# dbolya/yolact

Measured on AMD Instinct MI355X. Metric: images/sec (550x550, batch 8 per GPU), YOLACT yolact_resnet50 forward + Detect (Fast NMS), higher is better.
Workload: dtype f32 (fp32 in / fp32 accumulate / fp32 out; 92 % of the GEMM time on fp16x2 tiles = every fp32 operand as two fp16 pieces by round to nearest (22 significant bits + 2 signs: exact for ~2/3 of all fp32 values, one fp32 ulp otherwise), 3 exact piece products per product on the fp16 matrix pipe; measure

## Files before the change

### include/yolact_amd.h

```cpp
#ifndef YOLACT_AMD_H
#define YOLACT_AMD_H
#include <stddef.h>
#include <stdint.h>

#ifdef __cplusplus
extern "C" {
#endif

#define YMI_ABI_VERSION 9

#define YMI_EFORMAT (-4)
#define YMI_EUNSUPPORTED (-5)

enum { YMI_ACT_NONE = 0, YMI_ACT_RELU = 1, YMI_ACT_LEAKY01 = 2, YMI_ACT_TANH = 3, YMI_ACT_SIGMOID = 4 };
enum { YMI_RES_NONE = 0, YMI_RES_ADD = 1, YMI_RES_BILINEAR = 2 };

typedef struct {
  int32_t n0, n1;
  int32_t act;
  int32_t row_stride;
  int64_t batch_stride;
  float *ptr;
} ymi_conv_seg;

typedef struct {
  const float *x;
  const float *w;
  const float *scale;
  const float *bias;
  const float *res;
  int32_t B, H, W, Cin, ldx;
  int32_t Ho, Wo, Cout;
  int32_t kh, kw, stride, pad;
  int32_t Kpad;
  int32_t res_mode;
  int32_t res_ld;
  int32_t res_H, res_W;
  int32_t res_after_act;
  int32_t nseg;
  int32_t tile;
  int32_t cin_alg;
  int32_t split_k;
  ymi_conv_seg seg[3];
  const void *w_x3;
  float *split_ws;
  int32_t cout_alg;
  int32_t _pad2;
  const void *w_h2;
  const float *scale_h2;
  const float *winv_h2;
  const float *x_amax;
  float *y_amax;
  float x_amax_mul;
  int32_t _pad3;
} ymi_conv_desc;

enum { YMI_TILE_AUTO = 0, YMI_TILE_128x128 = 1, YMI_TILE_128x64 = 2, YMI_TILE_64x64 = 3, YMI_TILE_128x32 = 4,
       YMI_TILE_64x128 = 5, YMI_TILE_32x32_K4 = 6, YMI_TILE_64x32_K2 = 7, YMI_TILE_32x64_K2 = 8,
       YMI_TILE_64x64_S3 = 9, YMI_TILE_64x64_S4 = 10, YMI_TILE_64x128_S3 = 11, YMI_TILE_128x64_S3 = 12,
       YMI_TILE_32x32_K4_S4 = 13, YMI_TILE_64x32_K2_S3 = 14, YMI_TILE_32x64_K2_S3 = 15,
       YMI_TILE_128x128_W8 = 16, YMI_TILE_256x128_W8 = 17, YMI_TILE_128x256_W8 = 18,
       YMI_TILE_128x128_S3 = 19, YMI_TILE_128x128_W8_S3 = 20, YMI_TILE_256x128_W8_S3 = 21, YMI_TILE_128x128_W8_S4 = 22,
       YMI_TILE_WG_128x256 = 23,
       YMI_TILE_X3 = 32,
       YMI_TILE_H2 = 64,
       YMI_TILE_DCNP = 128 };
enum { YMI_DCNP_64x128 = 1, YMI_DCNP_64x128_W8 = 2, YMI_DCNP_64x64 = 3, YMI_DCNP_128x128_W8 = 4, YMI_DCNP_128x64_W8 = 5,
       YMI_DCNP_32x128 = 6,
       YMI_DCNP_96x128_W6 = 7, YMI_DCNP_128x128_W8_R1 = 8, YMI_DCNP_160x128_W10 = 9, YMI_DCNP_192x128_W12 = 10,
       YMI_DCNP_64x256_W8 = 11, YMI_DCNP_96x256_W12 = 12, YMI_DCNP_128x256_W16 = 13,
       YMI_DCNP_128x256_W8T = 14, YMI_DCNP_128x128_W4T = 15, YMI_DCNP_256x128_W8T = 16,
       YMI_DCNP_128x32_W4 = 17, YMI_DCNP_256x32_W8 = 18, YMI_DCNP_64x32_W2 = 19,
       YMI_DCNP_WS_128x32_W4 = 20, YMI_DCNP_WS_256x32_W8 = 21, YMI_DCNP_WS_256x32_W4 = 22, YMI_DCNP_WS_512x32_W8 = 23,
       YMI_DCNP_WS_128x64_W4 = 24, YMI_DCNP_WS_256x64_W8 = 25, YMI_DCNP_WS_256x64_W4 = 26, YMI_DCNP_WS_512x64_W8 = 27,
       YMI_DCNP_PATCH_C64 = 28,
       YMI_DCNP_PC_128x128 = 29,
       YMI_DCNP_PATCH2_256 = 30, YMI_DCNP_PATCH2_192 = 31 };

int ymi_abi_version(void);
const char *ymi_strerror(int code);

int ymi_conv2d_nhwc_f32(const ymi_conv_desc *d, void *stream);
double ymi_conv_flops(const ymi_conv_desc *d);
int ymi_conv_pick_tile(const ymi_conv_desc *d);

typedef struct {
  const float *x;
  const float *u;
  const float *scale;
  const float *bias;
  float *y;
  float *V, *M;
  int32_t B, H, W, C, Cout;
  int32_t act;
  int32_t tile;
  int32_t nseg;
  int32_t m;
  int32_t _pad0;
  ymi_conv_seg seg[3];
  const void *u_x3;
  int32_t cout_alg;
  int32_t v_planes;
  const void *u_h2;
  const float *uinv_h2;
  const float *x_amax;
  float *y_amax;
  const float *x_up;
  int32_t up_relu, _pad4;
  const void *proj_w_h2;
  const float *proj_scale_h2, *proj_bias;
  float *proj_y, *proj_y_amax;
  int32_t proj_cout, proj_ldy, proj_act, _pad5;
} ymi_wino_desc;
int ymi_conv3x3_winograd_f32(const ymi_wino_desc *d, void *stream);

#define YMI_AMAX_SUB 16
#define YMI_AMAX_STRIDE 64
int ymi_amax_f32(const float *x, long n, float *out, void *stream);

int ymi_nchw_to_nhwc4_f32(const float *x, float *y, int B, int C, int H, int W, void *stream);
int ymi_nchw_to_nhwc4_amax_f32(const float *x, float *y, int B, int C, int H, int W, float *amax, void *stream);
int ymi_nhwc_to_nchw_f32(const float *x, float *y, int B, int C, int H, int W, void *stream);
int ymi_maxpool3x3s2_nhwc_f32(const float *x, float *y, int B, int H, int W, int C, int Ho, int Wo, void *stream);
int ymi_bilinear_nhwc_f32(const float *x, float *y, int B, int Hi, int Wi, int C, int Ho, int Wo,
                          float scale_h, float scale_w, int relu, void *stream);

int ymi_bilinear_add_nhwc_f32(const float *x, float *y, int B, int Hi, int Wi, int C, int Ho, int Wo, float *y_amax, void *stream);

int ymi_conv2d_direct_nhwc_f32(const float *x, const float *w, const float *bias, float *y, int B, int H, int W,
                               int Cin, int Ho, int Wo, int Cout, int kh, int kw, int stride, int pad, int relu,
                               void *stream);
int ymi_global_maxpool_nhwc_f32(const float *x, float *y, int B, int HW, int C, void *stream);

typedef struct {
  const float *conf;
  const float *loc;
  const float *coef;
  const float *priors;
  int32_t B, P, C, D;
  int32_t conf_is_logits;
  int32_t top_k;
  int32_t max_det;
  float conf_thresh;
  float nms_thresh;
  int32_t cross_class;
  int32_t conf_ld;
  int32_t _pad1;
  float *scores_t;
  int32_t *keep;
  int32_t *num_keep;
  float *maxsc;
  int32_t *argmax;
  float *cand_score;
  int32_t *cand_prior;
  int32_t *out_count;
  float *out_box;
  float *out_score;
  int64_t *out_class;
  float *out_coef;
  int32_t *out_prior;
  float *out_rec;
} ymi_detect_desc;
int ymi_detect_f32(const ymi_detect_desc *d, void *stream);

typedef struct {
  float box_scale;
  int32_t _pad0;
  void *ws;
} ymi_detect_greedy_ws;
int ymi_detect_traditional_f32(const ymi_detect_desc *d, const ymi_detect_greedy_ws *g, void *stream);

int ymi_lincomb_crop_f32(const float *proto, const float *coef, const float *box, float *masks_lo,
                         int ph, int pw, int D, int N, int crop, void *stream);
int ymi_mask_upsample_f32(const float *masks_lo, float *out, int N, int ph, int pw, int h, int w,
                          float thresh, void *stream);
int ymi_lincomb_crop_batch_f32(const float *proto, const float *coef, const float *box, const int32_t *count,
                               float *masks_lo, int B, int cap, int ph, int pw, int D, int crop, void *stream);
int ymi_mask_upsample_batch_f32(const float *masks_lo, const int32_t *count, float *out, int B, int cap, int ph, int pw,
                                int h, int w, float thresh, void *stream);
enum { YMI_UP_FLAT = 1, YMI_UP_BAND = 2, YMI_UP_ROWS16 = 3, YMI_UP_ROWS32 = 4 };
int ymi_mask_upsample_kernel(int nmask, int ph, int pw, int h, int w, uintptr_t out_addr, int has_count);
int ymi_boxes_to_pixels(const float *box, int64_t *out, int N, int w, int h, void *stream);

int ymi_fast_base_transform_f32(const float *img, float *out, int N, int H, int W, int oh, int ow,
                                const float *mean_bgr, const float *std_bgr, int mode, int out_nhwc4, void *stream);

enum { YMI_AUG_PHOTOMETRIC = 1, YMI_AUG_BRIGHTNESS = 2, YMI_AUG_CONTRAST = 4, YMI_AUG_CONTRAST_LAST = 8, YMI_AUG_SATURATION = 16,
       YMI_AUG_HUE = 32, YMI_AUG_MIRROR = 64, YMI_AUG_SRC_F32 = 128 };
typedef struct ymi_augment_rec {
  const void *src;
  const uint8_t *masks;
  int32_t h, w, n_inst, flags;
  int32_t canvas_h, canvas_w, off_x, off_y;
  int32_t crop_x0, crop_y0, crop_x1, crop_y1;
  float delta, alpha, sat, hue;
  int32_t out_slot, mask_first, n_kept, kept_first;
} ymi_augment_rec;
typedef struct ymi_augment_desc {
  const ymi_augment_rec *recs;
  const int32_t *kept;
  float *out;
  void *masks_out;
  void *ws;
  int64_t ws_bytes;
  int32_t B, S, n_masks, mode, out_nhwc4, masks_u8;
  float mean_bgr[3], std_bgr[3];
} ymi_augment_desc;
int ymi_ssd_augment_f32(const ymi_augment_desc *d, void *stream);

int ymi_mask_iou_f32(const float *masks_a, const float *masks_b, int A, int B, long n, int iscrowd, float *ws, float *iou,
                     void *stream);

int ymi_jaccard_f32(const float *box_a, const float *box_b, int A, int B, int iscrowd, float *out, void *stream);
int ymi_mask_bits_f32(const float *masks, int N, long n, uint64_t *bits, void *stream);
int ymi_mask_upsample_bits(const float *masks_lo, int N, int ph, int pw, int h, int w, float thresh, uint64_t *bits, void *stream);
int ymi_mask_iou_bits(const uint64_t *bits_a, const uint64_t *bits_b, int A, int B, long W64, int iscrowd, float *iou, void *stream);

#define YMI_AP_NUM_THRESH 10
#define YMI_AP_MAX_DET 1024
#define YMI_AP_MAX_GT 2048
typedef struct {
  const int64_t *cls;
  const float *box_score;
  const float *mask_score;
  const float *box_iou;
  const float *mask_iou;
  const float *crowd_box_iou;
  const float *crowd_mask_iou;
  const int32_t *gt_cls;
  const int32_t *crowd_cls;
  int64_t *rec_key;
  float *rec_score;
  int32_t *rec_flags;
  int64_t *gt_count;
  int64_t base, cap;
  int32_t N, G, Gc, num_classes;
} ymi_ap_match_desc;
typedef struct {
  const int64_t *sorted_key;
  const int64_t *perm;
  const int32_t *rec_flags;
  const int64_t *gt_count;
  double *ap;
  int32_t *empty;
  int64_t M, cap;
  int32_t num_classes, _pad0;
} ymi_ap_finalize_desc;
int ymi_ap_match_f32(const ymi_ap_match_desc *d, void *stream);
int ymi_ap_finalize_f64(const ymi_ap_finalize_desc *d, void *stream);

int ymi_composite_masks_u8(const float *img, const float *masks, const float *colors, int n, int h, int w, float alpha,
                           unsigned char *out, void *stream);

int ymi_mask_rle_f32(const float *masks, int N, int h, int w, uint32_t *counts, int32_t *nruns, int cap, void *stream);
int ymi_mask_rle_upsampled_f32(const float *masks_lo, int N, int ph, int pw, int h, int w, float thresh, uint32_t *counts,
                               int32_t *nruns, int cap, void *stream);
int ymi_rle_to_string(const uint32_t *counts, const int32_t *nruns, int N, int cap, uint8_t *str, int32_t *nchars,
                      int cap_chars, void *stream);

enum { YMI_JPEG_YCBCR = 0, YMI_JPEG_RGB = 1, YMI_JPEG_GRAY = 2 };
typedef struct {
  int32_t width, height;
  int32_t ncomp;
  int32_t progressive;
  int32_t orientation;
// ... 442 lines not shown
```

### yolact_amd/_lib.py

```python
from __future__ import annotations

import ctypes as C
import os

_HERE = os.path.dirname(os.path.abspath(__file__))
LIB_PATH = os.path.join(_HERE, 'libyolact_amd.so')

ABI_VERSION = 9

ACT_NONE, ACT_RELU, ACT_LEAKY01, ACT_TANH, ACT_SIGMOID = 0, 1, 2, 3, 4
RES_NONE, RES_ADD, RES_BILINEAR = 0, 1, 2
TILE_AUTO, TILE_128x128, TILE_128x64, TILE_64x64, TILE_128x32, TILE_64x128 = 0, 1, 2, 3, 4, 5
TILE_32x32_K4, TILE_64x32_K2, TILE_32x64_K2 = 6, 7, 8
TILE_64x64_S3, TILE_64x64_S4, TILE_64x128_S3, TILE_128x64_S3, TILE_32x32_K4_S4, TILE_64x32_K2_S3, TILE_32x64_K2_S3 = range(9, 16)
TILE_NAMES = {1: '128x128', 2: '128x64', 3: '64x64', 4: '128x32', 5: '64x128', 6: '32x32k4', 7: '64x32k2', 8: '32x64k2',
              9: '64x64s3', 10: '64x64s4', 11: '64x128s3', 12: '128x64s3', 13: '32x32k4s4', 14: '64x32k2s3', 15: '32x64k2s3',
              16: '128x128w8', 17: '256x128w8', 18: '128x256w8', 19: '128x128s3', 20: '128x128w8s3', 21: '256x128w8s3',
              22: '128x128w8s4'}
TILE_128x128_W8, TILE_256x128_W8, TILE_128x256_W8 = 16, 17, 18
TILE_128x128_S3, TILE_128x128_W8_S3, TILE_256x128_W8_S3, TILE_128x128_W8_S4 = 19, 20, 21, 22
TILE_WG_128x256 = 23
TILE_X3 = 32
X3_BASE_TILES = (1, 2, 3, 5, 6, 7, 8, 9, 11, 12, 16, 17, 19, 20, 21, 22)
for _t in X3_BASE_TILES:
    TILE_NAMES[_t | TILE_X3] = TILE_NAMES[_t] + 'x3'
BASIC_TILES = (1, 2, 3, 4, 5)
TILE_H2 = 64
H2_BASE_TILES = X3_BASE_TILES + (18, 13, 14, 15)
for _t in H2_BASE_TILES:
    TILE_NAMES[_t | TILE_H2] = TILE_NAMES[_t] + 'h2'
TILE_NAMES[TILE_WG_128x256 | TILE_H2] = 'wg128x256h2'
TILE_DCNP = 128
DCNP_64x128, DCNP_64x128_W8, DCNP_64x64, DCNP_128x128_W8, DCNP_128x64_W8, DCNP_32x128 = 1, 2, 3, 4, 5, 6
DCNP_96x128_W6, DCNP_128x128_W8_R1, DCNP_160x128_W10, DCNP_192x128_W12, DCNP_64x256_W8, DCNP_96x256_W12, DCNP_128x256_W16 = range(7, 14)
DCNP_TILES = {1: 'dcnp64x128', 2: 'dcnp64x128w8', 3: 'dcnp64x64', 4: 'dcnp128x128w8', 5: 'dcnp128x64w8', 6: 'dcnp32x128',
              7: 'dcnp96x128w6', 8: 'dcnp128x128w8r1', 9: 'dcnp160x128w10', 10: 'dcnp192x128w12',
              11: 'dcnp64x256w8', 12: 'dcnp96x256w12', 13: 'dcnp128x256w16',
              14: 'dcnp128x256w8t', 15: 'dcnp128x128w4t', 16: 'dcnp256x128w8t',
              17: 'dcnp128x32w4', 18: 'dcnp256x32w8', 19: 'dcnp64x32w2'}
DCNP_128x32_W4, DCNP_256x32_W8, DCNP_64x32_W2 = 17, 18, 19
DCNP_PLAIN_ONLY = (14, 15, 16, 17, 18, 19)
WS_TILES = {20: 'ws128x32w4', 21: 'ws256x32w8', 22: 'ws256x32w4', 23: 'ws512x32w8',
            24: 'ws128x64w4', 25: 'ws256x64w8', 26: 'ws256x64w4', 27: 'ws512x64w8'}
DCNP_WS_128x32_W4, DCNP_WS_512x64_W8 = 20, 27
DCNP_PATCH_C64 = 28
PATCH_TILES = {28: 'patch8x16c64'}
PC_TILES = {29: 'pc128x128'}
DCNP_PC_128x128 = 29
PATCH2_TILES = {30: 'patch2p256', 31: 'patch2p192'}
DCNP_PATCH2_256, DCNP_PATCH2_192 = 30, 31
for _t, _n in list(DCNP_TILES.items()) + list(WS_TILES.items()) + list(PATCH_TILES.items()) + list(PC_TILES.items()) + list(PATCH2_TILES.items()):
    TILE_NAMES[_t | TILE_H2 | TILE_DCNP] = _n
WINO_PLANES = 1024
KSPLIT_TILES = (6, 7, 8, 13, 14, 15, 6 | 32, 7 | 32, 8 | 32, 6 | 64, 7 | 64, 8 | 64, 13 | 64, 14 | 64, 15 | 64)
AMAX_SLOT_FLOATS = 16 * 64


class ConvSeg(C.Structure):
    _fields_ = [('n0', C.c_int32), ('n1', C.c_int32), ('act', C.c_int32), ('row_stride', C.c_int32),
                ('batch_stride', C.c_int64), ('ptr', C.c_void_p)]


class ConvDesc(C.Structure):
    _fields_ = [('x', C.c_void_p), ('w', C.c_void_p), ('scale', C.c_void_p), ('bias', C.c_void_p),
                ('res', C.c_void_p),
                ('B', C.c_int32), ('H', C.c_int32), ('W', C.c_int32), ('Cin', C.c_int32), ('ldx', C.c_int32),
                ('Ho', C.c_int32), ('Wo', C.c_int32), ('Cout', C.c_int32),
                ('kh', C.c_int32), ('kw', C.c_int32), ('stride', C.c_int32), ('pad', C.c_int32),
                ('Kpad', C.c_int32), ('res_mode', C.c_int32), ('res_ld', C.c_int32),
                ('res_H', C.c_int32), ('res_W', C.c_int32), ('res_after_act', C.c_int32),
                ('nseg', C.c_int32), ('tile', C.c_int32), ('cin_alg', C.c_int32), ('split_k', C.c_int32),
                ('seg', ConvSeg * 3), ('w_x3', C.c_void_p), ('split_ws', C.c_void_p), ('cout_alg', C.c_int32),
                ('_pad2', C.c_int32),
                ('w_h2', C.c_void_p), ('scale_h2', C.c_void_p), ('winv_h2', C.c_void_p), ('x_amax', C.c_void_p),
                ('y_amax', C.c_void_p), ('x_amax_mul', C.c_float), ('_pad3', C.c_int32)]


class WinoDesc(C.Structure):
    _fields_ = [('x', C.c_void_p), ('u', C.c_void_p), ('scale', C.c_void_p), ('bias', C.c_void_p), ('y', C.c_void_p),
                ('V', C.c_void_p), ('M', C.c_void_p),
                ('B', C.c_int32), ('H', C.c_int32), ('W', C.c_int32), ('C', C.c_int32), ('Cout', C.c_int32),
                ('act', C.c_int32), ('tile', C.c_int32), ('nseg', C.c_int32), ('m', C.c_int32), ('_pad0', C.c_int32),
                ('seg', ConvSeg * 3), ('u_x3', C.c_void_p), ('cout_alg', C.c_int32), ('v_planes', C.c_int32),
                ('u_h2', C.c_void_p), ('uinv_h2', C.c_void_p), ('x_amax', C.c_void_p), ('y_amax', C.c_void_p),
                ('x_up', C.c_void_p), ('up_relu', C.c_int32), ('_pad4', C.c_int32),
                ('proj_w_h2', C.c_void_p), ('proj_scale_h2', C.c_void_p), ('proj_bias', C.c_void_p),
                ('proj_y', C.c_void_p), ('proj_y_amax', C.c_void_p),
                ('proj_cout', C.c_int32), ('proj_ldy', C.c_int32), ('proj_act', C.c_int32), ('_pad5', C.c_int32)]


class DcnDesc(C.Structure):
    _fields_ = [('conv', ConvDesc), ('offmask', C.c_void_p), ('ldo', C.c_int32), ('mask_is_prob', C.c_int32),
                ('om_layout', C.c_int32), ('_pad1', C.c_int32)]


class DcnBwdDesc(C.Structure):
    _fields_ = [('x', C.c_void_p), ('offmask', C.c_void_p), ('w', C.c_void_p), ('gy', C.c_void_p),
                ('gx', C.c_void_p), ('g_offset', C.c_void_p), ('g_mask', C.c_void_p), ('gw', C.c_void_p), ('gbias', C.c_void_p),
                ('B', C.c_int32), ('H', C.c_int32), ('W', C.c_int32), ('Cin', C.c_int32), ('ldx', C.c_int32),
                ('Ho', C.c_int32), ('Wo', C.c_int32), ('Cout', C.c_int32),
                ('kh', C.c_int32), ('kw', C.c_int32), ('stride', C.c_int32), ('pad', C.c_int32), ('dilation', C.c_int32),
                ('deformable_groups', C.c_int32),
                ('ldo', C.c_int32), ('mask_is_prob', C.c_int32), ('om_layout', C.c_int32), ('_pad0', C.c_int32)]


class DcnColsDesc(C.Structure):
    _fields_ = [('x', C.c_void_p), ('om', C.c_void_p), ('col', C.c_void_p), ('dcol', C.c_void_p), ('g_om', C.c_void_p),
                ('gx', C.c_void_p), ('keys', C.c_void_p), ('coef', C.c_void_p), ('sorted_keys', C.c_void_p), ('order', C.c_void_p),
                ('seg', C.c_void_p),
                ('B', C.c_int32), ('H', C.c_int32), ('W', C.c_int32), ('Cin', C.c_int32), ('Ho', C.c_int32), ('Wo', C.c_int32),
                ('stride', C.c_int32), ('_pad0', C.c_int32)]


class MaskLossDesc(C.Structure):
    _fields_ = [('proto', C.c_void_p), ('coef', C.c_void_p), ('box', C.c_void_p), ('gt', C.c_void_p), ('gt_idx', C.c_void_p),
                ('img_off', C.c_void_p), ('weight', C.c_void_p),
                ('loss', C.c_void_p), ('loss_inst', C.c_void_p), ('d_proto', C.c_void_p), ('d_coef', C.c_void_p), ('ws', C.c_void_p),
                ('B', C.c_int32), ('mh', C.c_int32), ('mw', C.c_int32), ('K', C.c_int32), ('N', C.c_int32), ('G', C.c_int32),
                ('crop', C.c_int32), ('roi_norm', C.c_int32), ('alpha', C.c_float), ('_pad0', C.c_int32)]


class MatchDesc(C.Structure):
    _fields_ = [('priors', C.c_void_p), ('truth', C.c_void_p), ('label', C.c_void_p), ('gt_off', C.c_void_p),
                ('gt_off_host', C.c_void_p), ('crowd', C.c_void_p), ('crowd_off', C.c_void_p), ('crowd_off_host', C.c_void_p),
                ('loc_data', C.c_void_p), ('loc_t', C.c_void_p), ('gt_box_t', C.c_void_p), ('conf_t', C.c_void_p),
                ('idx_t', C.c_void_p), ('pos', C.c_void_p), ('num_pos', C.c_void_p), ('d_loc', C.c_void_p), ('loss', C.c_void_p),
                ('ws', C.c_void_p),
                ('B', C.c_int32), ('P', C.c_int32), ('G', C.c_int32), ('Gc', C.c_int32),
                ('pos_thresh', C.c_float), ('neg_thresh', C.c_float), ('crowd_thresh', C.c_float), ('bbox_alpha', C.c_float)]


class ClassLossDesc(C.Structure):
    _fields_ = [('conf', C.c_void_p), ('conf_t', C.c_void_p), ('loss', C.c_void_p), ('neg', C.c_void_p), ('num_neg', C.c_void_p),
                ('d_conf', C.c_void_p), ('ws', C.c_void_p),
                ('B', C.c_int32), ('P', C.c_int32), ('C', C.c_int32), ('negpos_ratio', C.c_int32), ('conf_alpha', C.c_float),
                ('_pad0', C.c_int32)]


class SegmLossDesc(C.Structure):
    _fields_ = [('segm', C.c_void_p), ('gt', C.c_void_p), ('label', C.c_void_p), ('gt_off', C.c_void_p), ('gt_off_host', C.c_void_p),
                ('loss', C.c_void_p), ('d_segm', C.c_void_p), ('ws', C.c_void_p),
                ('B', C.c_int32), ('K', C.c_int32), ('mh', C.c_int32), ('mw', C.c_int32), ('G', C.c_int32), ('alpha', C.c_float)]


class MaskIouInputDesc(C.Structure):
    _fields_ = [('proto', C.c_void_p), ('coef', C.c_void_p), ('box', C.c_void_p), ('gt', C.c_void_p), ('gt_idx', C.c_void_p),
                ('img_off', C.c_void_p), ('img_off_host', C.c_void_p), ('x0', C.c_void_p), ('iou_t', C.c_void_p),
                ('d_x0', C.c_void_p), ('d_proto', C.c_void_p), ('d_coef', C.c_void_p), ('ws', C.c_void_p), ('ws_bytes', C.c_int64),
                ('B', C.c_int32), ('mh', C.c_int32), ('mw', C.c_int32), ('K', C.c_int32), ('N', C.c_int32), ('G', C.c_int32)]


class ConvBwdDesc(C.Structure):
    _fields_ = [('x', C.c_void_p), ('w', C.c_void_p), ('y', C.c_void_p), ('dy', C.c_void_p), ('dx', C.c_void_p), ('dw', C.c_void_p),
                ('db', C.c_void_p), ('ws', C.c_void_p), ('ws_bytes', C.c_int64),
                ('B', C.c_int32), ('H', C.c_int32), ('W', C.c_int32), ('Cin', C.c_int32), ('Ho', C.c_int32), ('Wo', C.c_int32),
                ('Cout', C.c_int32), ('kh', C.c_int32), ('kw', C.c_int32), ('stride', C.c_int32), ('pad', C.c_int32),
                ('relu', C.c_int32)]


class MaskIouHeadDesc(C.Structure):
    _fields_ = [('pool', C.c_void_p), ('iou_t', C.c_void_p), ('label', C.c_void_p), ('loss', C.c_void_p), ('d_pool', C.c_void_p),
                ('ws', C.c_void_p), ('ws_bytes', C.c_int64), ('N', C.c_int32), ('C', C.c_int32), ('alpha', C.c_float),
                ('_pad0', C.c_int32)]


class ConvWgradDesc(C.Structure):
    _fields_ = [('x', C.c_void_p), ('g', C.c_void_p), ('dw', C.c_void_p), ('db', C.c_void_p), ('ws', C.c_void_p),
                ('ws_bytes', C.c_int64),
                ('B', C.c_int32), ('H', C.c_int32), ('W', C.c_int32), ('Cin', C.c_int32), ('Cout', C.c_int32), ('ldg', C.c_int32),
                ('kh', C.c_int32), ('kw', C.c_int32), ('pad', C.c_int32), ('stride', C.c_int32)]


class ConvDgradDesc(C.Structure):
    _fields_ = [('g', C.c_void_p), ('w', C.c_void_p), ('dx', C.c_void_p),
                ('B', C.c_int32), ('H', C.c_int32), ('W', C.c_int32), ('Cin', C.c_int32), ('Cout', C.c_int32), ('ldg', C.c_int32),
                ('kh', C.c_int32), ('kw', C.c_int32), ('pad', C.c_int32), ('stride', C.c_int32)]


class ConvPackDesc(C.Structure):
    _fields_ = [('w', C.c_void_p * 3), ('planes', C.c_void_p), ('winv', C.c_void_p), ('w32', C.c_void_p),
                ('cout', C.c_int32 * 3), ('n', C.c_int32), ('Cin', C.c_int32), ('k', C.c_int32), ('mode', C.c_int32), ('ld', C.c_int32)]


class BnDesc(C.Structure):
    _fields_ = [('x', C.c_void_p), ('res', C.c_void_p), ('gamma', C.c_void_p), ('beta', C.c_void_p),
                ('running_mean', C.c_void_p), ('running_var', C.c_void_p), ('y', C.c_void_p), ('mean', C.c_void_p),
                ('invstd', C.c_void_p), ('dy', C.c_void_p), ('dx', C.c_void_p), ('d_res', C.c_void_p), ('dgamma', C.c_void_p),
                ('dbeta', C.c_void_p), ('ws', C.c_void_p), ('ws_bytes', C.c_int64), ('npos', C.c_int64),
                ('C', C.c_int32), ('training', C.c_int32), ('relu', C.c_int32), ('eps', C.c_float), ('momentum', C.c_float),
                ('_pad0', C.c_int32)]


class StemWgradDesc(C.Structure):
    _fields_ = [('x', C.c_void_p), ('g', C.c_void_p), ('dw', C.c_void_p), ('ws', C.c_void_p), ('ws_bytes', C.c_int64),
                ('B', C.c_int32), ('H', C.c_int32), ('W', C.c_int32), ('Cout', C.c_int32), ('ldg', C.c_int32), ('_pad0', C.c_int32)]


class PreconvWgradDesc(C.Structure):
    _fields_ = [('x', C.c_void_p), ('g', C.c_void_p), ('dw', C.c_void_p), ('ws', C.c_void_p), ('ws_bytes', C.c_int64),
                ('B', C.c_int32), ('H', C.c_int32), ('W', C.c_int32), ('Cout', C.c_int32), ('ldg', C.c_int32), ('_pad0', C.c_int32)]


AUG_PHOTOMETRIC, AUG_BRIGHTNESS, AUG_CONTRAST, AUG_CONTRAST_LAST, AUG_SATURATION, AUG_HUE, AUG_MIRROR, AUG_SRC_F32 = (
    1, 2, 4, 8, 16, 32, 64, 128)


class AugmentRec(C.Structure):
    _fields_ = [('src', C.c_void_p), ('masks', C.c_void_p),
                ('h', C.c_int32), ('w', C.c_int32), ('n_inst', C.c_int32), ('flags', C.c_int32),
                ('canvas_h', C.c_int32), ('canvas_w', C.c_int32), ('off_x', C.c_int32), ('off_y', C.c_int32),
                ('crop_x0', C.c_int32), ('crop_y0', C.c_int32), ('crop_x1', C.c_int32), ('crop_y1', C.c_int32),
                ('delta', C.c_float), ('alpha', C.c_float), ('sat', C.c_float), ('hue', C.c_float),
                ('out_slot', C.c_int32), ('mask_first', C.c_int32), ('n_kept', C.c_int32), ('kept_first', C.c_int32)]


class AugmentDesc(C.Structure):
    _fields_ = [('recs', C.POINTER(AugmentRec)), ('kept', C.c_void_p), ('out', C.c_void_p), ('masks_out', C.c_void_p),
                ('ws', C.c_void_p), ('ws_bytes', C.c_int64),
                ('B', C.c_int32), ('S', C.c_int32), ('n_masks', C.c_int32), ('mode', C.c_int32), ('out_nhwc4', C.c_int32),
                ('masks_u8', C.c_int32), ('mean_bgr', C.c_float * 3), ('std_bgr', C.c_float * 3)]


COCO_POLY, COCO_COUNTS = 0, 1
COCO_MASK_MAX_PIXELS = 640000


class CocoMaskRec(C.Structure):
    _fields_ = [('out', C.c_void_p), ('kind', C.c_int32), ('h', C.c_int32), ('w', C.c_int32), ('n', C.c_int32),
                ('first', C.c_int32), ('xy_first', C.c_int32)]


class CocoMaskDesc(C.Structure):
    _fields_ = [('recs', C.POINTER(CocoMaskRec)), ('xy', C.c_void_p), ('poly_len', C.c_void_p), ('counts', C.c_void_p),
                ('ws', C.c_void_p), ('ws_bytes', C.c_int64),
                ('n_vert', C.c_int64), ('n_poly', C.c_int64), ('n_counts', C.c_int64), ('n', C.c_int32), ('_pad0', C.c_int32)]


SGD_CHUNK = 4096


class SgdTensor(C.Structure):
# ... 253 lines not shown
```

### yolact_amd/csrc/api.cpp

```cpp
#include "../../include/yolact_amd.h"
#include <hip/hip_runtime_api.h>

extern "C" {

int64_t ymi_detect_greedy_layout(const ymi_detect_desc *d, int64_t off[4]);
int64_t ymi_jpeg_enc_layout(int h, int w, int sub, int64_t off[8], int64_t *out_bound);
int64_t ymi_mask_loss_ws_bytes(const ymi_mask_loss_desc *d);
int64_t ymi_match_ws_bytes(const ymi_match_desc *d);
int64_t ymi_box_loss_ws_bytes(const ymi_match_desc *d);
int64_t ymi_class_loss_ws_bytes(const ymi_class_loss_desc *d);
int64_t ymi_segm_loss_ws_bytes(const ymi_segm_loss_desc *d);
int64_t ymi_maskiou_input_ws_bytes(const ymi_maskiou_input_desc *d);
int64_t ymi_conv_bwd_ws_bytes(const ymi_conv_bwd_desc *d);
int64_t ymi_maskiou_head_ws_bytes(const ymi_maskiou_head_desc *d);
int64_t ymi_conv_wgrad_ws_bytes(const ymi_conv_wgrad_desc *d);
int64_t ymi_bn_ws_bytes(const ymi_bn_desc *d);
int64_t ymi_stem_wgrad_ws_bytes(const ymi_stem_wgrad_desc *d);
int64_t ymi_augment_ws_bytes(const ymi_augment_desc *d);
int64_t ymi_preconv_wgrad_ws_bytes(const ymi_preconv_wgrad_desc *d);
int64_t ymi_conv_wgrad_h2_ws_bytes(const ymi_conv_wgrad_desc *d);
int64_t ymi_coco_mask_ws_bytes(const ymi_coco_mask_desc *d);

int ymi_abi_version(void) { return YMI_ABI_VERSION; }

const char *ymi_strerror(int code) {
  switch (code) {
    case 0: return "ok";
    case -1: return "bad argument / unsupported configuration";
    case -2: return "shape or alignment constraint violated";
    case -3: return "null pointer";
    case YMI_EFORMAT: return "corrupt or truncated input stream";
    case YMI_EUNSUPPORTED: return "valid input outside the supported subset";
  }
  if (code > 0) return hipGetErrorString((hipError_t)code);
  return "unknown error";
}

int64_t ymi_workspace_bytes(int what, const void *desc) {
  auto cdiv = [](int64_t a, int64_t b) { return (a + b - 1) / b; };
  if (what == YMI_WS_AMAX_SLOT) return (int64_t)YMI_AMAX_SUB * YMI_AMAX_STRIDE * 4;
  if (!desc) return -3;
  switch (what) {
    case YMI_WS_WINO_V:
    case YMI_WS_WINO_M: {
      const ymi_wino_desc *d = (const ymi_wino_desc *)desc;
      const int m = d->m == 4 ? 4 : 2;
      if ((d->m != 0 && d->m != 2 && d->m != 4) || d->B < 1 || d->H < 1 || d->W < 1 || d->C < 1 || d->Cout < 1) return -1;
      const int64_t G = (int64_t)(m + 2) * (m + 2), T = (int64_t)d->B * cdiv(d->H, m) * cdiv(d->W, m);
      return 4 * G * T * (what == YMI_WS_WINO_V ? (int64_t)d->C : cdiv(d->Cout, 4) * 4);
    }
    case YMI_WS_SPLITK: {
      const ymi_conv_desc *d = (const ymi_conv_desc *)desc;
      if (d->B < 1 || d->Ho < 1 || d->Wo < 1 || d->Cout < 1 || d->split_k < 0) return -1;
      return d->split_k > 1 ? 4 * (int64_t)d->split_k * d->B * d->Ho * d->Wo * d->Cout : 0;
    }
    case YMI_WS_MASK_IOU: {
      const ymi_mask_iou_shape *d = (const ymi_mask_iou_shape *)desc;
      if (d->A < 0 || d->B < 0) return -1;
      return 4 * ((int64_t)d->A * d->B + d->A + d->B);
    }
    case YMI_WS_JPEG_COEFS: return 2 * ((const ymi_jpeg_info *)desc)->coef_count;
    case YMI_WS_JPEG_PLANES: return ((const ymi_jpeg_info *)desc)->plane_bytes;
    case YMI_WS_DETECT_SCORES_T:
    case YMI_WS_DETECT_PER_PRIOR:
    case YMI_WS_DETECT_CAND:
    case YMI_WS_DETECT_REC: {
      const ymi_detect_desc *d = (const ymi_detect_desc *)desc;
      if (d->B < 1 || d->P < 1 || d->C < 2 || d->D < 0 || d->top_k < 1 || d->max_det < 1) return -1;
      if (what == YMI_WS_DETECT_SCORES_T) return 4 * (int64_t)d->B * (d->C - 1) * d->P;
      if (what == YMI_WS_DETECT_PER_PRIOR) return 4 * (int64_t)d->B * d->P;
      if (what == YMI_WS_DETECT_CAND) return 4 * (int64_t)d->B * (d->C - 1) * d->top_k;
      const int64_t cap = d->cross_class ? d->top_k : d->max_det;
      return 4 * (int64_t)d->B * (1 + cap * (6 + d->D));
    }
    case YMI_WS_DETECT_GREEDY: {
      const ymi_detect_desc *d = (const ymi_detect_desc *)desc;
      if (d->B < 1 || d->P < 1 || d->C < 2 || d->max_det < 1) return -1;
      int64_t off[4];
      return ymi_detect_greedy_layout(d, off);
    }
    case YMI_WS_JPEG_ENC:
    case YMI_WS_JPEG_ENC_OUT: {
      const ymi_jpeg_enc_desc *d = (const ymi_jpeg_enc_desc *)desc;
      int64_t off[8], bound = 0;
      const int64_t total = ymi_jpeg_enc_layout(d->h, d->w, d->subsampling, off, &bound);
      return total < 0 ? total : (what == YMI_WS_JPEG_ENC ? total : bound);
    }
    case YMI_WS_MASK_LOSS: return ymi_mask_loss_ws_bytes((const ymi_mask_loss_desc *)desc);
    case YMI_WS_MATCH: return ymi_match_ws_bytes((const ymi_match_desc *)desc);
    case YMI_WS_BOX_LOSS: return ymi_box_loss_ws_bytes((const ymi_match_desc *)desc);
    case YMI_WS_CLASS_LOSS: return ymi_class_loss_ws_bytes((const ymi_class_loss_desc *)desc);
    case YMI_WS_SEGM_LOSS: return ymi_segm_loss_ws_bytes((const ymi_segm_loss_desc *)desc);
    case YMI_WS_MASKIOU_INPUT: return ymi_maskiou_input_ws_bytes((const ymi_maskiou_input_desc *)desc);
    case YMI_WS_CONV_BWD: return ymi_conv_bwd_ws_bytes((const ymi_conv_bwd_desc *)desc);
    case YMI_WS_MASKIOU_HEAD: return ymi_maskiou_head_ws_bytes((const ymi_maskiou_head_desc *)desc);
    case YMI_WS_CONV_WGRAD: return ymi_conv_wgrad_ws_bytes((const ymi_conv_wgrad_desc *)desc);
    case YMI_WS_BN: return ymi_bn_ws_bytes((const ymi_bn_desc *)desc);
    case YMI_WS_STEM_WGRAD: return ymi_stem_wgrad_ws_bytes((const ymi_stem_wgrad_desc *)desc);
    case YMI_WS_AUGMENT: return ymi_augment_ws_bytes((const ymi_augment_desc *)desc);
    case YMI_WS_PRECONV_WGRAD: return ymi_preconv_wgrad_ws_bytes((const ymi_preconv_wgrad_desc *)desc);
    case YMI_WS_CONV_WGRAD_H2: return ymi_conv_wgrad_h2_ws_bytes((const ymi_conv_wgrad_desc *)desc);
    case YMI_WS_COCO_MASK: return ymi_coco_mask_ws_bytes((const ymi_coco_mask_desc *)desc);
    case YMI_WS_RLE_COUNTS: {
      const ymi_rle_shape *d = (const ymi_rle_shape *)desc;
      if (d->N < 0 || d->h < 1 || d->w < 1) return -1;
      const int64_t cap = d->cap > 0 ? d->cap : (int64_t)d->h * d->w + 1;
      return 4 * (int64_t)d->N * cap;
    }
  }
  return -1;
}

}
```

### yolact_amd/csrc/winograd.hip

```cpp
#include "gemm_h2.h"

int ymi_internal_grouped_gemm(const ymi_conv_desc *d, int groups, long x_gs, long w_gs, long y_gs, double prof_flops,
                              int prof_kind, hipStream_t s, const void *a2 = nullptr, unsigned a2_plane = 0, long a2_gs = 0,
                              unsigned sc_gs = 0);
int ymi_internal_wgemm(const void *v, const void *u, const float *uinv, const float *x_amax, float amax_mul, float *m, int G, long T,
                       int C, int Ng, int cout_pad, double prof_flops, int prof_kind, hipStream_t s);
int ymi_internal_prof_begin(double flops, int tile, int kind, hipStream_t s);
void ymi_internal_prof_end(int idx, hipStream_t s);

namespace {

typedef _Float16 f16x4 __attribute__((ext_vector_type(4)));

__device__ __forceinline__ void store_v_planes(_Float16 *o, long e, long stride_e2, long plane, const f32x4 v, float s) {
  f16x4 h, l;
#pragma unroll
  for (int k = 0; k < 4; ++k) {
    const float t = v[k] * s;
    h[k] = (_Float16)t;
    l[k] = (_Float16)(t - (float)h[k]);
  }
  *reinterpret_cast<f16x4 *>(o + e * stride_e2) = h;
  *reinterpret_cast<f16x4 *>(o + e * stride_e2 + plane) = l;
}
// ... 109 lines not shown

__device__ __forceinline__ float wino_act(float v, int act) {
  switch (act) {
    case YMI_ACT_RELU: return v > 0.f ? v : 0.f;
    case YMI_ACT_LEAKY01: return v > 0.f ? v : 0.1f * v;
    case YMI_ACT_TANH: return tanhf(v);
    case YMI_ACT_SIGMOID: return 1.f / (1.f + expf(-v));
    default: return v;
  }
}

__device__ __forceinline__ int seg_vec4(const SegTab &st, int n, int Cout) {
  if (n + 3 >= Cout) return -1;
#pragma unroll
  for (int k = 0; k < 3; ++k)
    if (k < st.nseg && n >= st.seg[k].n0 && n + 3 < st.seg[k].n1 && ((n - st.seg[k].n0) & 3) == 0 &&
        (st.seg[k].row_stride & 3) == 0 && (st.seg[k].batch_stride & 3) == 0 && (((uintptr_t)st.seg[k].ptr) & 15) == 0)
      return k;
  return -1;
}

struct SegVec {
  float *ptr; long bs; int rs, act;
  f32x4 sc, bi;
};
__device__ __forceinline__ SegVec seg_vec_setup(const SegTab &st, int k, const float *__restrict__ scale,
                                                const float *__restrict__ bias, int n) {
  ymi_conv_seg sg = st.seg[0];
  if (k == 1) sg = st.seg[1];
  if (k == 2) sg = st.seg[2];
  SegVec v;
  v.ptr = sg.ptr + (n - sg.n0); v.bs = sg.batch_stride; v.rs = sg.row_stride; v.act = sg.act;
#pragma unroll
  for (int e = 0; e < 4; ++e) { v.sc[e] = scale ? scale[n + e] : 1.f; v.bi[e] = bias ? bias[n + e] : 0.f; }
  return v;
}

constexpr int YMI_AMAX_SLOT = YMI_AMAX_SUB * YMI_AMAX_STRIDE;
__device__ __forceinline__ void seg_amax_add(float (&am)[3], int k, float v) {
  am[0] = k == 0 ? fmaxf(am[0], v) : am[0];
  am[1] = k == 1 ? fmaxf(am[1], v) : am[1];
  am[2] = k == 2 ? fmaxf(am[2], v) : am[2];
}
__device__ __forceinline__ void seg_amax_commit(float *y_amax, int nseg, const ymi_amax_pre &apre0, const float (&am)[3]) {
  if (!y_amax) return;
  ymi_amax_finish(apre0, am[0]);
  if (nseg > 1) ymi_amax_finish(ymi_amax_prefetch(y_amax + YMI_AMAX_SLOT), am[1]);
  if (nseg > 2) ymi_amax_finish(ymi_amax_prefetch(y_amax + 2 * YMI_AMAX_SLOT), am[2]);
}

__device__ __forceinline__ float seg_vec_store(const SegVec &sv, f32x4 v, long b, long pix) {
  v = v * sv.sc + sv.bi;
  if (sv.act <= YMI_ACT_LEAKY01) {
    const float slope = ymi_act_slope(sv.act);
#pragma unroll
    for (int e = 0; e < 4; ++e) v[e] = fmaxf(v[e], slope * v[e]);
  } else {
#pragma unroll
    for (int e = 0; e < 4; ++e) v[e] = wino_act(v[e], sv.act);
  }
  *reinterpret_cast<f32x4 *>(sv.ptr + b * sv.bs + pix * sv.rs) = v;
  return ymi_absmax4(v);
}

__global__ __launch_bounds__(256) void wino_out_seg_k(const float *__restrict__ Mm, const SegTab st,
                                                      const float *__restrict__ scale, const float *__restrict__ bias,
                                                      int Ho, int Wo, int N4, int Cout, int th, int tw, long T, long total, float *__restrict__ y_amax) {
  float am[3] = {0.f, 0.f, 0.f};
  const ymi_amax_pre apre = ymi_amax_prefetch(y_amax);
  for (unsigned i = blockIdx.x * 256u + threadIdx.x; i < (unsigned)total; i += gridDim.x * 256u) {
    const unsigned tu = i / (unsigned)N4, ru = tu / (unsigned)tw, bu = ru / (unsigned)th;
    const int n4 = (int)(i - tu * (unsigned)N4), tx = (int)(tu - ru * (unsigned)tw), ty = (int)(ru - bu * (unsigned)th);
    const long t = tu, b = bu;
    const long stride_e = T * (N4 * 4L);
    const float *src = Mm + t * (N4 * 4L) + n4 * 4;
    f32x4 m[4][4];
#pragma unroll
    for (int e = 0; e < 16; ++e) m[e >> 2][e & 3] = *reinterpret_cast<const f32x4 *>(src + e * stride_e);
    f32x4 s[2][4];
#pragma unroll
    for (int j = 0; j < 4; ++j) {
      s[0][j] = (m[0][j] + m[1][j]) + m[2][j];
      s[1][j] = (m[1][j] - m[2][j]) - m[3][j];
    }
    f32x4 o[2][2];
#pragma unroll
    for (int iy = 0; iy < 2; ++iy) {
      o[iy][0] = (s[iy][0] + s[iy][1]) + s[iy][2];
      o[iy][1] = (s[iy][1] - s[iy][2]) - s[iy][3];
    }
    const int kv = seg_vec4(st, n4 * 4, Cout);
    if (kv >= 0) {
      const SegVec sv = seg_vec_setup(st, kv, scale, bias, n4 * 4);
#pragma unroll
      for (int iy = 0; iy < 2; ++iy)
#pragma unroll
        for (int ix = 0; ix < 2; ++ix) {
          const int oy = 2 * ty + iy, ox = 2 * tx + ix;
          if (oy < Ho && ox < Wo) seg_amax_add(am, kv, seg_vec_store(sv, o[iy][ix], b, (long)oy * Wo + ox));
        }
      continue;
    }
#pragma unroll
    for (int e = 0; e < 4; ++e) {
      const int n = n4 * 4 + e;
      if (n >= Cout) continue;
      float *ptr = nullptr; long bs = 0; int rs = 0, act = 0, n0 = 0, ks = 0;
#pragma unroll
      for (int k = 0; k < 3; ++k)
        if (k < st.nseg && n >= st.seg[k].n0 && n < st.seg[k].n1) {
          ptr = st.seg[k].ptr; bs = st.seg[k].batch_stride; rs = st.seg[k].row_stride; act = st.seg[k].act; n0 = st.seg[k].n0; ks = k;
        }
      if (!ptr) continue;
      const float sc = scale ? scale[n] : 1.f, bi = bias ? bias[n] : 0.f;
#pragma unroll
      for (int iy = 0; iy < 2; ++iy) {
        const int oy = 2 * ty + iy;
        if (oy >= Ho) continue;
#pragma unroll
        for (int ix = 0; ix < 2; ++ix) {
          const int ox = 2 * tx + ix;
          if (ox >= Wo) continue;
          const float val = wino_act(o[iy][ix][e] * sc + bi, act);
          seg_amax_add(am, ks, fabsf(val));
          ptr[b * bs + ((long)oy * Wo + ox) * rs + (n - n0)] = val;
        }
      }
    }
  }
  seg_amax_commit(y_amax, st.nseg, apre, am);
}


__device__ __forceinline__ void bt6(const f32x4 v0, const f32x4 v1, const f32x4 v2, const f32x4 v3, const f32x4 v4, const f32x4 v5,
                                    f32x4 &t0, f32x4 &t1, f32x4 &t2, f32x4 &t3, f32x4 &t4, f32x4 &t5) {
  const f32x4 a = v4 - v2 * 4.f, b = v3 - v1 * 4.f;
  const f32x4 c = v4 - v2, e = (v3 - v1) * 2.f;
  t0 = (v0 * 4.f - v2 * 5.f) + v4;
  t1 = a + b;
  t2 = a - b;
  t3 = c + e;
  t4 = c - e;
  t5 = (v1 * 4.f - v3 * 5.f) + v5;
}

__device__ __forceinline__ void up2_coord(int dst, int in_size, float &l1) {
  float src = 0.5f * ((float)dst + 0.5f) - 0.5f;
  src = src < 0.f ? 0.f : src;
  int i0 = (int)src;
  if (i0 > in_size - 1) i0 = in_size - 1;
  l1 = src - (float)i0;
}

template <bool PLANES, bool UPS = false>
__global__ __launch_bounds__(256) void wino43_in_k(const float *__restrict__ x, float *__restrict__ V, int H, int W, int C4,
                                                   int th, int tw, long T, long total, const float *__restrict__ x_amax,
                                                   int up_relu = 0) {
  float vs = 1.f, vinv = 1.f;
  if (PLANES) ymi_h2_scale(ymi_amax_read(x_amax) * 100.f, vs, vinv);
  for (unsigned i = blockIdx.x * 256u + threadIdx.x; i < (unsigned)total; i += gridDim.x * 256u) {
    const unsigned tu = i / (unsigned)C4, ru = tu / (unsigned)tw, bu = ru / (unsigned)th;
    const int c4 = (int)(i - tu * (unsigned)C4), tx = (int)(tu - ru * (unsigned)tw), ty = (int)(ru - bu * (unsigned)th);
    const long t = tu, b = bu;
    const int y0 = 4 * ty - 1, x0 = 4 * tx - 1;
    f32x4 u[6][6];
    if constexpr (UPS) {
      const int Hl = H >> 1, Wl = W >> 1;
      const float *lbase = x + ((b * Hl) * (long)Wl) * (C4 * 4L) + c4 * 4;
      f32x4 lo[4][4];
#pragma unroll
      for (int k = 0; k < 4; ++k) {
        int wy = 2 * ty - 1 + k; wy = wy < 0 ? 0 : (wy > Hl - 1 ? Hl - 1 : wy);
#pragma unroll
        for (int q = 0; q < 4; ++q) {
          int wx = 2 * tx - 1 + q; wx = wx < 0 ? 0 : (wx > Wl - 1 ? Wl - 1 : wx);
          lo[k][q] = *reinterpret_cast<const f32x4 *>(lbase + ((long)wy * Wl + wx) * (C4 * 4L));
        }
      }
      float lx[6], ly[6];
#pragma unroll
      for (int j = 0; j < 6; ++j) { up2_coord(x0 + j, Wl, lx[j]); up2_coord(y0 + j, Hl, ly[j]); }
      f32x4 hrow[4][6];
#pragma unroll
      for (int k = 0; k < 4; ++k)
#pragma unroll
        for (int j = 0; j < 6; ++j) hrow[k][j] = (1.f - lx[j]) * lo[k][j >> 1] + lx[j] * lo[k][(j >> 1) + 1];
#pragma unroll
      for (int j = 0; j < 6; ++j) {
        const bool xok = (unsigned)(x0 + j) < (unsigned)W;
        f32x4 dcol[6];
#pragma unroll
        for (int iy = 0; iy < 6; ++iy) {
          const bool ok = xok && (unsigned)(y0 + iy) < (unsigned)H;
          f32x4 v = (1.f - ly[iy]) * hrow[iy >> 1][j] + ly[iy] * hrow[(iy >> 1) + 1][j];
          if (up_relu) {
#pragma unroll
            for (int e = 0; e < 4; ++e) v[e] = v[e] < 0.f ? 0.f : v[e];
          }
          const f32x4 z = {0.f, 0.f, 0.f, 0.f};
          dcol[iy] = ok ? v : z;
        }
        bt6(dcol[0], dcol[1], dcol[2], dcol[3], dcol[4], dcol[5], u[0][j], u[1][j], u[2][j], u[3][j], u[4][j], u[5][j]);
      }
    } else {
    const float *base = x + ((b * H) * (long)W) * (C4 * 4L) + c4 * 4;
#pragma unroll
    for (int j = 0; j < 6; ++j) {
      const int xx = x0 + j;
      const bool xok = (unsigned)xx < (unsigned)W;
      f32x4 dcol[6];
#pragma unroll
      for (int iy = 0; iy < 6; ++iy) {
        const int yy = y0 + iy;
        const bool ok = xok && (unsigned)yy < (unsigned)H;
        dcol[iy] = ld4(base + ((long)(ok ? yy : 0) * W + (ok ? xx : 0)) * (C4 * 4L), ok);
      }
      bt6(dcol[0], dcol[1], dcol[2], dcol[3], dcol[4], dcol[5], u[0][j], u[1][j], u[2][j], u[3][j], u[4][j], u[5][j]);
    }
    }
    const long stride_e = T * (C4 * 4L);
    float *o = V + t * (C4 * 4L) + c4 * 4;
    _Float16 *o2 = reinterpret_cast<_Float16 *>(V) + t * (C4 * 4L) + c4 * 4;
#pragma unroll
    for (int iy = 0; iy < 6; ++iy) {
      f32x4 v[6];
      bt6(u[iy][0], u[iy][1], u[iy][2], u[iy][3], u[iy][4], u[iy][5], v[0], v[1], v[2], v[3], v[4], v[5]);
#pragma unroll
      for (int l = 0; l < 6; ++l) {
        if (PLANES) store_v_planes(o2, iy * 6 + l, 2 * stride_e, stride_e, v[l], vs);
        else *reinterpret_cast<f32x4 *>(o + (iy * 6 + l) * stride_e) = v[l];
      }
    }
  }
}

__device__ __forceinline__ void at6(const f32x4 v0, const f32x4 v1, const f32x4 v2, const f32x4 v3, const f32x4 v4, const f32x4 v5,
                                    f32x4 &s0, f32x4 &s1, f32x4 &s2, f32x4 &s3) {
  const f32x4 p12 = v1 + v2, m12 = v1 - v2, p34 = v3 + v4, m34 = v3 - v4;
  s0 = (v0 + p12) + p34;
  s1 = m12 + m34 * 2.f;
  s2 = p12 + p34 * 4.f;
  s3 = (m12 + m34 * 8.f) + v5;
}

__device__ __forceinline__ void wino43_out_tile(const float *__restrict__ src, long stride_e, f32x4 (&o)[4][4]) {
  f32x4 s[4][6];
#pragma unroll
  for (int j = 0; j < 6; ++j) {
    f32x4 mc[6];
#pragma unroll
    for (int iy = 0; iy < 6; ++iy) mc[iy] = *reinterpret_cast<const f32x4 *>(src + (iy * 6 + j) * stride_e);
    at6(mc[0], mc[1], mc[2], mc[3], mc[4], mc[5], s[0][j], s[1][j], s[2][j], s[3][j]);
  }
#pragma unroll
  for (int iy = 0; iy < 4; ++iy) at6(s[iy][0], s[iy][1], s[iy][2], s[iy][3], s[iy][4], s[iy][5], o[iy][0], o[iy][1], o[iy][2], o[iy][3]);
}

__global__ __launch_bounds__(256) void wino43_out_k(const float *__restrict__ Mm, float *__restrict__ y,
                                                    const float *__restrict__ scale, const float *__restrict__ bias, int Ho,
                                                    int Wo, int N4, int th, int tw, long T, int act, long total,
                                                    float *__restrict__ y_amax) {
  float am = 0.f;
  const ymi_amax_pre apre = ymi_amax_prefetch(y_amax);
  for (unsigned i = blockIdx.x * 256u + threadIdx.x; i < (unsigned)total; i += gridDim.x * 256u) {
    const unsigned tu = i / (unsigned)N4, ru = tu / (unsigned)tw, bu = ru / (unsigned)th;
    const int n4 = (int)(i - tu * (unsigned)N4), tx = (int)(tu - ru * (unsigned)tw), ty = (int)(ru - bu * (unsigned)th);
    const long t = tu, b = bu;
    f32x4 o[4][4];
    wino43_out_tile(Mm + t * (N4 * 4L) + n4 * 4, T * (N4 * 4L), o);
    f32x4 sc = {1.f, 1.f, 1.f, 1.f}, bi = {0.f, 0.f, 0.f, 0.f};
    if (scale) sc = *reinterpret_cast<const f32x4 *>(scale + n4 * 4);
    if (bias) bi = *reinterpret_cast<const f32x4 *>(bias + n4 * 4);
    const float slope = ymi_act_slope(act);
#pragma unroll
    for (int iy = 0; iy < 4; ++iy)
#pragma unroll
      for (int ix = 0; ix < 4; ++ix) {
        f32x4 v = o[iy][ix] * sc + bi;
#pragma unroll
        for (int e = 0; e < 4; ++e) v[e] = fmaxf(v[e], slope * v[e]);
        o[iy][ix] = v;
        const bool ok = 4 * ty + iy < Ho && 4 * tx + ix < Wo;
        am = fmaxf(am, ok ? ymi_absmax4(v) : 0.f);
      }
#pragma unroll
    for (int iy = 0; iy < 4; ++iy)
#pragma unroll
      for (int ix = 0; ix < 4; ++ix) {
        const int oy = 4 * ty + iy, ox = 4 * tx + ix;
        if (oy < Ho && ox < Wo) *reinterpret_cast<f32x4 *>(y + ((b * Ho + oy) * (long)Wo + ox) * (N4 * 4L) + n4 * 4) = o[iy][ix];
      }
  }
  if (y_amax) ymi_amax_finish(apre, am);
}

struct ProjArgs {
  const void *w_h2; const float *scale_h2, *bias; float *y, *y_amax;
  int cout, ldy, act; unsigned w_plane;
};
constexpr int PJ_ROW = 528, PJ_YPLANE = 16 * PJ_ROW, PJ_WPLANE = 32 * PJ_ROW, PJ_LDS = 2 * PJ_WPLANE + 4 * 2 * PJ_YPLANE;

__global__ __launch_bounds__(256) void wino43_out_proj_k(const float *__restrict__ Mm, const float *__restrict__ scale,
                                                         const float *__restrict__ bias, int Ho, int Wo, int th, int tw, long T,
                                                         int act, const ProjArgs pp) {
#if defined(__HIP_DEVICE_COMPILE__)
  __shared__ __attribute__((aligned(16))) char lds[PJ_LDS];
  typedef _Float16 f16x8 __attribute__((ext_vector_type(8)));
  typedef _Float16 f16x4 __attribute__((ext_vector_type(4)));
  const int t = threadIdx.x, lane = t & 63, wave = __builtin_amdgcn_readfirstlane(t >> 6);
  const int lr = lane & 15, g = lane >> 4;
  const ymi_amax_pre apre = ymi_amax_prefetch(pp.y_amax);
  for (int u = t; u < 2 * 32 * 32; u += 256) {
    const int plane = u >> 10, row = (u >> 5) & 31, pc = u & 31;
    const f32x4 v = *reinterpret_cast<const f32x4 *>(reinterpret_cast<const char *>(pp.w_h2) + (size_t)plane * pp.w_plane + (size_t)row * 512 + pc * 16);
    *reinterpret_cast<f32x4 *>(lds + plane * PJ_WPLANE + row * PJ_ROW + pc * 16) = v;
  }
  __syncthreads();
  char *ytile = lds + 2 * PJ_WPLANE + wave * (2 * PJ_YPLANE);
  f32x4 sc = {1.f, 1.f, 1.f, 1.f}, bi = {0.f, 0.f, 0.f, 0.f};
  if (scale) sc = *reinterpret_cast<const f32x4 *>(scale + lane * 4);
  if (bias) bi = *reinterpret_cast<const f32x4 *>(bias + lane * 4);
  const float slope = ymi_act_slope(act);
  const float slope2 = ymi_act_slope(pp.act);
  float am = 0.f;
  for (long tl = (long)blockIdx.x * 4 + wave; tl < T; tl += (long)gridDim.x * 4) {
    const unsigned tu = (unsigned)tl, ru = tu / (unsigned)tw, bu = ru / (unsigned)th;
    const int tx = (int)(tu - ru * (unsigned)tw), ty = (int)(ru - bu * (unsigned)th);
    f32x4 o[4][4];
    wino43_out_tile(Mm + tl * 256L + lane * 4, T * 256L, o);
    float tm = 0.f;
#pragma unroll
    for (int iy = 0; iy < 4; ++iy)
#pragma unroll
      for (int ix = 0; ix < 4; ++ix) {
        f32x4 v = o[iy][ix] * sc + bi;
#pragma unroll
        for (int e = 0; e < 4; ++e) v[e] = fmaxf(v[e], slope * v[e]);
        o[iy][ix] = v;
        tm = fmaxf(tm, ymi_absmax4(v));
      }
    const unsigned tmb = ymi_wave_umax63(__builtin_bit_cast(unsigned, tm));
    float sT, invT;
    ymi_h2_scale(__builtin_bit_cast(float, (unsigned)__builtin_amdgcn_readlane((int)tmb, 63)), sT, invT);
#pragma unroll
    for (int iy = 0; iy < 4; ++iy)
#pragma unroll
      for (int ix = 0; ix < 4; ++ix) {
        const f32x4 v = o[iy][ix] * sT;
        f16x4 h4, l4;
#pragma unroll
        for (int e = 0; e < 4; ++e) {
          const _Float16 h = (_Float16)v[e];
          h4[e] = h;
          l4[e] = (_Float16)(v[e] - (float)h);
        }
        char *dst = ytile + (iy * 4 + ix) * PJ_ROW + lane * 8;
        *reinterpret_cast<f16x4 *>(dst) = h4;
        *reinterpret_cast<f16x4 *>(dst + PJ_YPLANE) = l4;
      }
    __builtin_amdgcn_fence(__ATOMIC_RELEASE, "wavefront");
    __builtin_amdgcn_wave_barrier();
    f32x4 acc[2];
    acc[0] = f32x4{0.f, 0.f, 0.f, 0.f};
    acc[1] = f32x4{0.f, 0.f, 0.f, 0.f};
#pragma unroll
    for (int c = 0; c < 8; ++c) {
      const f16x8 xh = *reinterpret_cast<const f16x8 *>(ytile + lr * PJ_ROW + c * 64 + g * 16);
      const f16x8 xl = *reinterpret_cast<const f16x8 *>(ytile + PJ_YPLANE + lr * PJ_ROW + c * 64 + g * 16);
#pragma unroll
      for (int j = 0; j < 2; ++j) {
        const f16x8 wh = *reinterpret_cast<const f16x8 *>(lds + (j * 16 + lr) * PJ_ROW + c * 64 + g * 16);
        const f16x8 wl = *reinterpret_cast<const f16x8 *>(lds + PJ_WPLANE + (j * 16 + lr) * PJ_ROW + c * 64 + g * 16);
        acc[j] = ymi_mfma16(wl, xh, acc[j]);
        acc[j] = ymi_mfma16(wh, xl, acc[j]);
        acc[j] = ymi_mfma16(wh, xh, acc[j]);
      }
    }
    __builtin_amdgcn_fence(__ATOMIC_ACQUIRE, "wavefront");
    __builtin_amdgcn_wave_barrier();
    const int oy = 4 * ty + (lr >> 2), ox = 4 * tx + (lr & 3);
#pragma unroll
    for (int j = 0; j < 2; ++j) {
      const int n = j * 16 + 4 * g;
      if (n < pp.cout && oy < Ho && ox < Wo) {
        f32x4 v;
#pragma unroll
        for (int e = 0; e < 4; ++e) {
          const float r = acc[j][e] * (pp.scale_h2[n + e] * invT) + (pp.bias ? pp.bias[n + e] : 0.f);
          v[e] = fmaxf(r, slope2 * r);
        }
        am = fmaxf(am, ymi_absmax4(v));
        *reinterpret_cast<f32x4 *>(pp.y + (((long)bu * Ho + oy) * (long)Wo + ox) * pp.ldy + n) = v;
      }
    }
  }
  if (pp.y_amax) ymi_amax_finish(apre, am);
#endif
}

__global__ __launch_bounds__(256) void wino43_out_seg_k(const float *__restrict__ Mm, const SegTab st,
                                                        const float *__restrict__ scale, const float *__restrict__ bias,
                                                        int Ho, int Wo, int N4, int Cout, int th, int tw, long T, long total, float *__restrict__ y_amax) {
  float am[3] = {0.f, 0.f, 0.f};
  const ymi_amax_pre apre = ymi_amax_prefetch(y_amax);
  for (unsigned i = blockIdx.x * 256u + threadIdx.x; i < (unsigned)total; i += gridDim.x * 256u) {
    const unsigned tu = i / (unsigned)N4, ru = tu / (unsigned)tw, bu = ru / (unsigned)th;
    const int n4 = (int)(i - tu * (unsigned)N4), tx = (int)(tu - ru * (unsigned)tw), ty = (int)(ru - bu * (unsigned)th);
    const long t = tu, b = bu;
    f32x4 o[4][4];
    wino43_out_tile(Mm + t * (N4 * 4L) + n4 * 4, T * (N4 * 4L), o);
    const int kv = seg_vec4(st, n4 * 4, Cout);
    if (kv >= 0) {
      const SegVec sv = seg_vec_setup(st, kv, scale, bias, n4 * 4);
#pragma unroll
      for (int iy = 0; iy < 4; ++iy)
#pragma unroll
        for (int ix = 0; ix < 4; ++ix) {
          const int oy = 4 * ty + iy, ox = 4 * tx + ix;
          if (oy < Ho && ox < Wo) seg_amax_add(am, kv, seg_vec_store(sv, o[iy][ix], b, (long)oy * Wo + ox));
        }
      continue;
    }
#pragma unroll
    for (int e = 0; e < 4; ++e) {
      const int n = n4 * 4 + e;
      if (n >= Cout) continue;
      float *ptr = nullptr; long bs = 0; int rs = 0, act = 0, n0 = 0, ks = 0;
#pragma unroll
      for (int k = 0; k < 3; ++k)
        if (k < st.nseg && n >= st.seg[k].n0 && n < st.seg[k].n1) {
          ptr = st.seg[k].ptr; bs = st.seg[k].batch_stride; rs = st.seg[k].row_stride; act = st.seg[k].act; n0 = st.seg[k].n0; ks = k;
        }
      if (!ptr) continue;
      const float sc = scale ? scale[n] : 1.f, bi = bias ? bias[n] : 0.f;
#pragma unroll
      for (int iy = 0; iy < 4; ++iy) {
        const int oy = 4 * ty + iy;
        if (oy >= Ho) continue;
#pragma unroll
        for (int ix = 0; ix < 4; ++ix) {
          const int ox = 4 * tx + ix;
          if (ox >= Wo) continue;
          const float val = wino_act(o[iy][ix][e] * sc + bi, act);
          seg_amax_add(am, ks, fabsf(val));
          ptr[b * bs + ((long)oy * Wo + ox) * rs + (n - n0)] = val;
        }
      }
    }
  }
  seg_amax_commit(y_amax, st.nseg, apre, am);
}

unsigned grid_for(long total) {
  long g = (total + 255) / 256;
  const long cap = 256L * 64;
  return (unsigned)(g > cap ? cap : g);
}

}

extern "C" int ymi_conv3x3_winograd_f32(const ymi_wino_desc *d, void *stream) {
  if (!d || (!d->x && !d->x_up) || !d->u || !d->V || !d->M) return YMI_ENULL;
  if (d->x_up && (d->m != 4 || (d->H & 1) || (d->W & 1) || (((uintptr_t)d->x_up) & 15))) return YMI_ESHAPE;
  if (d->B <= 0 || d->H <= 0 || d->W <= 0 || d->C <= 0 || d->Cout <= 0 || d->nseg < 0 || d->nseg > 3) return YMI_EARG;
  const bool proj = d->proj_w_h2 != nullptr;
  if (proj && (d->m != 4 || d->nseg != 0 || d->Cout != 256 || d->proj_cout <= 0 || d->proj_cout > 32 || (d->proj_cout & 3) ||
               (d->proj_ldy & 3) || d->proj_ldy < d->proj_cout || d->proj_act > YMI_ACT_LEAKY01 || d->proj_act < 0))
    return YMI_ESHAPE;
  if (proj && (!d->proj_scale_h2 || !d->proj_y || (((uintptr_t)d->proj_w_h2) & 15) || (((uintptr_t)d->proj_y) & 15))) return YMI_ENULL;
  if (d->nseg == 0 && ((!d->y && !proj) || (d->Cout & 3) || d->act > YMI_ACT_LEAKY01 || d->act < 0)) return YMI_ESHAPE;
  for (int k = 0; k < d->nseg; ++k) if (!d->seg[k].ptr) return YMI_ENULL;
  if (d->C & 31) return YMI_ESHAPE;
  if (d->m != 0 && d->m != 2 && d->m != 4) return YMI_EARG;
  const int mt = d->m == 4 ? 4 : 2;
  const int ng = (mt + 2) * (mt + 2);
  const int Ng = (d->Cout + 3) / 4 * 4;
  hipStream_t s = (hipStream_t)stream;
  const int th = (d->H + mt - 1) / mt, tw = (d->W + mt - 1) / mt;
  const long T = (long)d->B * th * tw;
  if (T * (long)(d->C > Ng ? d->C : Ng) >= (1L << 29)) return YMI_ESHAPE;
  const int C4 = d->C / 4, N4 = Ng / 4;
  const double alg = 2.0 * d->B * d->H * d->W * (double)(d->cout_alg > 0 ? d->cout_alg : d->Cout) * 9.0 * d->C;
  const double exe = 2.0 * ng * (double)T * d->C * Ng;
  const int outer = ymi_internal_prof_begin(alg, d->tile ? d->tile : YMI_TILE_64x64, mt == 4 ? 4 : 3, s);
  const bool h2 = (d->tile & YMI_TILE_H2) != 0;
  if (h2 && (!d->u_h2 || !d->uinv_h2 || !d->x_amax)) return YMI_ENULL;
  const bool planes = h2 && d->v_planes != 0;
#ifdef YMI_DIAGNOSTICS
  static const int wabl = [] { const char *e = getenv("YMI_WINO_ABLATE"); return e ? atoi(e) : 0; }();
  if (!(wabl & 1)) {
#endif
  if (mt == 4) {
    if (d->x_up) {
      if (planes) hipLaunchKernelGGL((wino43_in_k<true, true>), dim3(grid_for(T * C4)), dim3(256), 0, s, d->x_up, d->V, d->H, d->W, C4, th, tw, T, T * C4, d->x_amax, d->up_relu);
      else hipLaunchKernelGGL((wino43_in_k<false, true>), dim3(grid_for(T * C4)), dim3(256), 0, s, d->x_up, d->V, d->H, d->W, C4, th, tw, T, T * C4, d->x_amax, d->up_relu);
    } else if (planes) hipLaunchKernelGGL((wino43_in_k<true, false>), dim3(grid_for(T * C4)), dim3(256), 0, s, d->x, d->V, d->H, d->W, C4, th, tw, T, T * C4, d->x_amax, 0);
    else hipLaunchKernelGGL((wino43_in_k<false, false>), dim3(grid_for(T * C4)), dim3(256), 0, s, d->x, d->V, d->H, d->W, C4, th, tw, T, T * C4, d->x_amax, 0);
  } else {
    if (planes) hipLaunchKernelGGL(wino_in_k<true>, dim3(grid_for(T * C4)), dim3(256), 0, s, d->x, d->V, d->H, d->W, C4, th, tw, T, T * C4, d->x_amax);
    else hipLaunchKernelGGL(wino_in_k<false>, dim3(grid_for(T * C4)), dim3(256), 0, s, d->x, d->V, d->H, d->W, C4, th, tw, T, T * C4, d->x_amax);
  }
#ifdef YMI_DIAGNOSTICS
  }
#endif
  int rc = ymi_launch_status();
  if (rc) return rc;
  ymi_conv_desc g = {};
  g.x = d->V; g.w = d->u;
  g.B = 1; g.H = (int)T; g.W = 1; g.Cin = d->C; g.ldx = d->C;
  g.Ho = (int)T; g.Wo = 1; g.Cout = Ng;
  g.kh = g.kw = 1; g.stride = 1; g.pad = 0; g.Kpad = d->C;
  g.nseg = 1; g.tile = d->tile;
  g.w_x3 = d->u_x3;
  g.w_h2 = d->u_h2; g.scale_h2 = d->uinv_h2; g.winv_h2 = d->uinv_h2;
  g.x_amax = d->x_amax; g.x_amax_mul = mt == 4 ? 100.f : 4.f;
  g.seg[0].n0 = 0; g.seg[0].n1 = Ng; g.seg[0].act = YMI_ACT_NONE; g.seg[0].row_stride = Ng;
  g.seg[0].batch_stride = T * Ng; g.seg[0].ptr = d->M;
  const long cout_pad = ((long)d->Cout + 127) / 128 * 128;
  if ((d->tile & 31) == YMI_TILE_WG_128x256) {
    if (!planes || (d->tile & YMI_TILE_X3)) return YMI_EARG;
    rc = ymi_internal_wgemm(d->V, d->u_h2, d->uinv_h2, d->x_amax, mt == 4 ? 100.f : 4.f, d->M, ng, T, d->C, Ng, (int)cout_pad, exe,
                            mt == 4 ? 6 : 5, s);
  } else if (planes)
    rc = ymi_internal_grouped_gemm(&g, ng, T * d->C, cout_pad * d->C, T * Ng, exe, mt == 4 ? 6 : 5, s, d->V,
                                   (unsigned)(T * d->C * 2), 2L * T * d->C * 2, (unsigned)cout_pad);
  else
    rc = ymi_internal_grouped_gemm(&g, ng, T * d->C, cout_pad * d->C, T * Ng, exe, mt == 4 ? 6 : 5 , s,
                                   nullptr, 0, 0, (unsigned)cout_pad);
  if (rc) return rc;
  if (d->nseg > 0) {
    SegTab st;
    st.nseg = d->nseg;
    for (int k = 0; k < 3; ++k) st.seg[k] = d->seg[k];
    if (mt == 4)
      hipLaunchKernelGGL(wino43_out_seg_k, dim3(grid_for(T * N4)), dim3(256), 0, s, d->M, st, d->scale, d->bias, d->H, d->W,
                         N4, d->Cout, th, tw, T, T * N4, d->y_amax);
    else
      hipLaunchKernelGGL(wino_out_seg_k, dim3(grid_for(T * N4)), dim3(256), 0, s, d->M, st, d->scale, d->bias, d->H, d->W, N4,
                         d->Cout, th, tw, T, T * N4, d->y_amax);
    rc = ymi_launch_status();
    ymi_internal_prof_end(outer, s);
    return rc;
  }
  if (proj) {
    ProjArgs pa;
    pa.w_h2 = d->proj_w_h2; pa.scale_h2 = d->proj_scale_h2; pa.bias = d->proj_bias; pa.y = d->proj_y; pa.y_amax = d->proj_y_amax;
    pa.cout = d->proj_cout; pa.ldy = d->proj_ldy; pa.act = d->proj_act; pa.w_plane = (unsigned)(128L * 256 * 2);
    const long blocks = (T + 3) / 4;
    hipLaunchKernelGGL(wino43_out_proj_k, dim3((unsigned)(blocks < 256 ? blocks : 256)), dim3(256), 0, s, d->M, d->scale, d->bias, d->H,
                       d->W, th, tw, T, d->act, pa);
    rc = ymi_launch_status();
    ymi_internal_prof_end(outer, s);
    if (rc == YMI_OK) {
      const int pr = ymi_internal_prof_begin(2.0 * d->B * d->H * d->W * 256.0 * d->proj_cout, d->tile ? d->tile : YMI_TILE_64x64, 12, s);
      ymi_internal_prof_end(pr, s);
    }
    return rc;
  }
  if (mt == 4)
    hipLaunchKernelGGL(wino43_out_k, dim3(grid_for(T * N4)), dim3(256), 0, s, d->M, d->y, d->scale, d->bias, d->H, d->W, N4, th,
                       tw, T, d->act, T * N4, d->y_amax);
  else
    hipLaunchKernelGGL(wino_out_k, dim3(grid_for(T * N4)), dim3(256), 0, s, d->M, d->y, d->scale, d->bias, d->H, d->W, N4, th,
                       tw, T, d->act, T * N4, d->y_amax);
  rc = ymi_launch_status();
  ymi_internal_prof_end(outer, s);
  return rc;
}
```

### yolact_amd/engine.py

```python
from __future__ import annotations

import ctypes as C
import os
from typing import List, Optional

import torch
import torch.nn as nn

from . import _lib as L
from .config import act_name, make_priors_host
from . import modules as M
from .plan_tune import PlanTuning, _ceil


SPLIT_DEFAULT = '2'


def split3_planes(w: torch.Tensor) -> torch.Tensor:
    w = w.detach().to(torch.float32).contiguous()
    mask = -65536

    def hi(t):
        u = t.view(torch.int32) & mask
        return u.view(torch.float32), (u >> 16).to(torch.int16)
# ... 195 lines not shown

def pack_offmask(conv: nn.Conv2d, device, interleave: bool) -> Packed:
    w, b = conv.weight.detach().float(), conv.bias.detach().float()
    assert w.shape[0] == 27 and conv.stride[0] == conv.stride[1] and conv.padding == (1, 1), 'conv_offset_mask of a 3x3 one-group DCN'
    order = [c for k in range(9) for c in (2 * k, 2 * k + 1, 18 + k)] if interleave else list(range(27))
    wp, bp = w.new_zeros((32,) + tuple(w.shape[1:])), b.new_zeros(32)
    wp[:27], bp[:27] = w[order], b[order]
    pk = Packed(wp, bp, None, conv.stride[0], 1, None, device)
    pk.cout_alg = 27
    return pk


def pack_module(conv: nn.Conv2d, bn=None, device=None, cin_pad=None) -> Packed:
    assert conv.dilation == (1, 1) and conv.groups == 1
    assert conv.stride[0] == conv.stride[1] and conv.padding[0] == conv.padding[1]
    return Packed(conv.weight, conv.bias, bn, conv.stride[0], conv.padding[0], cin_pad, device)


class T:
    __slots__ = ('buf', 'B', 'H', 'W', 'C', 'slot', 'gain')

    def __init__(self, buf, B, H, W, C, slot=None, gain=None):
        self.buf, self.B, self.H, self.W, self.C = buf, B, H, W, C
        self.slot = slot
        self.gain = gain

    @property
    def ptr(self):
        return self.buf.data_ptr()

    def view(self):
        return self.buf[: self.B * self.H * self.W * self.C].view(self.B, self.H, self.W, self.C)


class Arena:

    def __init__(self, device):
        self.device = device
        self.free_list: List[torch.Tensor] = []
        self.all: List[torch.Tensor] = []

    def alloc(self, numel) -> torch.Tensor:
        best = None
        for i, b in enumerate(self.free_list):
            if b.numel() >= numel and (best is None or b.numel() < self.free_list[best].numel()):
                best = i
        if best is not None:
            return self.free_list.pop(best)
        b = torch.empty(numel, dtype=torch.float32, device=self.device)
        self.all.append(b)
        return b

    def free(self, t):
        if isinstance(t, _Borrowed):
            return
        buf = t.buf if isinstance(t, T) else t
        assert all(buf is not f for f in self.free_list)
        self.free_list.append(buf)

    def total_bytes(self):
        return sum(b.numel() * 4 for b in self.all)


def out_size(n, k, s, p):
    return (n + 2 * p - k) // s + 1


_SIDE_STREAMS = {}


def _side_stream(device):
    n = int(os.environ.get('YOLACT_AMD_SIDE_STREAMS', '2'))
    if n <= 0:
        return torch.cuda.Stream(device=device)
    pool = _side_pool(device, n)
    st = pool['streams'][pool['next'] % n]
    pool['next'] += 1
    return st


def _side_pool(device, n):
    key = (device.type, device.index if device.index is not None else torch.cuda.current_device())
    pool = _SIDE_STREAMS.get(key)
    if pool is None:
        pool = _SIDE_STREAMS[key] = {'streams': [torch.cuda.Stream(device=device) for _ in range(n)], 'next': 0}
    return pool


def side_stream_pool(device):
    n = int(os.environ.get('YOLACT_AMD_SIDE_STREAMS', '2'))
    return tuple(_side_pool(device, n)['streams']) if n > 0 else ()


class _OpList(list):
    version = 0

    def _bump(self):
        self.version += 1

    def __setitem__(self, k, v):
        self._bump(); list.__setitem__(self, k, v)

    def __delitem__(self, k):
        self._bump(); list.__delitem__(self, k)

    def append(self, v):
        self._bump(); list.append(self, v)

    def insert(self, k, v):
        self._bump(); list.insert(self, k, v)

    def pop(self, *a):
        self._bump(); return list.pop(self, *a)

    def extend(self, it):
        self._bump(); list.extend(self, it)


class Plan(PlanTuning):
    def __init__(self, net, B, H, W, device, dry_two_streams=False):
        self.net, self.B, self.H, self.W, self.device = net, B, H, W, device
        self.ops = _OpList()
        self.conv_meta = []
        self.arena = Arena(device)
        self.keepalive = []
        self.lib = L.lib()
        self.two_streams = (device.type == 'cuda' and os.environ.get('YOLACT_AMD_STREAMS', '2') != '1') or dry_two_streams
        self.stream_b = _side_stream(device) if self.two_streams and device.type == 'cuda' else None
        self.overlap = True
        self.events = {}
        self._cur = 'A'
        wsel = os.environ.get('YOLACT_AMD_WINOGRAD', '1')
        self.use_winograd = device.type == 'cuda' and wsel != '0'
        self.wino_variants = (2,) if wsel == '2' else (4,) if wsel == '4' else (2, 4)
        self.wino_force = os.environ.get('YOLACT_AMD_WINOGRAD_FORCE', '0') == '1'
        smode = os.environ.get('YOLACT_AMD_SPLIT', SPLIT_DEFAULT)
        self.split = smode == '1'
        self.h2 = smode == '2'
        self.mode = 'x3' if self.split else 'h2' if self.h2 else ''
        self.amax = torch.zeros(512 * L.AMAX_SLOT_FLOATS, dtype=torch.float32, device=device)
        self._nslots = 0
        self.splitk = os.environ.get('YOLACT_AMD_SPLITK', '1') == '1'
        self.pipe = os.environ.get('YOLACT_AMD_PIPE', '1') == '1'
        self.wide_guard = os.environ.get('YOLACT_AMD_WIDE_GUARD', '1') == '1'
        self.om_pad = os.environ.get('YOLACT_AMD_OM_PAD', '1') == '1'
        self.om_interleave = os.environ.get('YOLACT_AMD_OM_INTERLEAVE', '1') == '1'
        self.native_exec = device.type == 'cuda' and os.environ.get('YOLACT_AMD_NATIVE_EXEC', '1') == '1'
        self._native, self._native_events, self._stem_desc = None, None, None
        self.wide_ops = set()
        self.wide_layers = []
        self._sk_ws = {}
        self.down_on_side_stream = os.environ.get('YOLACT_AMD_DOWN_STREAM', 'B') == 'B'
        self.wino_alt, self._wino_packed, self._wino_ws = {}, {}, {}
        self._upsrc, self.wino_up = {}, {}
        self._done_event = None
        self._priors_timed = False
        self.param_stamp = None
        self.tune_misses = 0
        self._build()
        if self.wide_layers:
            import warnings
            warnings.warn('yolact_amd: %d layer(s) consume compensated OUTLIER channels (tiny filter columns on channels their producer '
                          'amplifies, Packed.tiny_columns) and run on bf16x3 / exact-fp32 tiles instead of fp16x2, without Winograd and '
                          'the fp16x2-only fusions: %s.  YOLACT_AMD_WIDE_GUARD=0 keeps fp16x2 (at reduced accuracy for such checkpoints).'
                          % (len(self.wide_layers), ', '.join(self.wide_layers[:12]) + (' ...' if len(self.wide_layers) > 12 else '')),
                          RuntimeWarning, stacklevel=2)
        self._bind_wino_workspaces()
        self.sections = [None if op[0] in ('record', 'wait', 'detect', 'nop') else self.section_of(op[2]) for op in self.ops]

    def _arena(self):
        if self._cur == 'B':
            if not hasattr(self, 'arena_b'):
                self.arena_b = Arena(self.device)
            return self.arena_b
        return self.arena

    def _new(self, B, H, W, C, slot=None, gain=None) -> T:
        return T(self._arena().alloc(B * H * W * C), B, H, W, C, slot, gain)

    def _slot(self):
        self._nslots += 1
        assert self._nslots * L.AMAX_SLOT_FLOATS <= self.amax.numel()
        return self._nslots - 1

    def _slot_ptr(self, slot):
        return self.amax.data_ptr() + 4 * L.AMAX_SLOT_FLOATS * slot

    def bound(self, slot):
        return float(self.amax[slot * L.AMAX_SLOT_FLOATS:(slot + 1) * L.AMAX_SLOT_FLOATS].max())

    def free(self, t):
        self._arena().free(t)

    def conv(self, name, x: T, pk: Packed, act=L.ACT_NONE, res: Optional[T] = None, res_mode=L.RES_NONE,
             res_after_act=0, out: Optional[T] = None, segs=None, dcn_offmask: Optional[T] = None) -> Optional[T]:
        assert x.C == pk.Cin, (name, x.C, pk.Cin)
        Ho, Wo = out_size(x.H, pk.kh, pk.stride, pk.pad), out_size(x.W, pk.kw, pk.stride, pk.pad)
        d = L.ConvDesc()
        d.x, d.w = x.ptr, pk.w.data_ptr()
        d.scale = pk.scale.data_ptr() if pk.scale is not None else None
        d.bias = pk.bias.data_ptr() if pk.bias is not None else None
        d.B, d.H, d.W, d.Cin, d.ldx = x.B, x.H, x.W, pk.Cin, x.C
        d.Ho, d.Wo, d.Cout = Ho, Wo, pk.Cout
        d.kh, d.kw, d.stride, d.pad, d.Kpad = pk.kh, pk.kw, pk.stride, pk.pad, pk.Kpad
        d.res_mode = res_mode
        d.res_after_act = res_after_act
        if res is not None:
            d.res, d.res_ld, d.res_H, d.res_W = res.ptr, res.C, res.H, res.W
            if res_mode == L.RES_ADD:
                assert (res.B, res.H, res.W, res.C) == (x.B, Ho, Wo, pk.Cout), name
        d.tile = L.TILE_AUTO
        d.cin_alg = pk.cin_alg
        d.cout_alg = pk.cout_alg
        wide = self.h2 and self.wide_guard and pk.Cin % 32 == 0 and pk.tiny_columns(in_gain=x.gain)
        pk.wide = wide
        if wide:
            self.wide_layers.append(name)
        og = pk.out_gain()
        if res is not None and res.gain is not None and res.gain.numel() == og.numel():
            og = torch.maximum(og, res.gain)
        self.last_out_gain = og
        if (self.split or wide) and dcn_offmask is None:
            d.w_x3 = pk.w3().data_ptr()
        yslot = self._slot()
        for _ in range(len(segs) - 1 if segs else 0):
            self._slot()
        if self.h2:
            d.y_amax = self._slot_ptr(yslot)
        if x.slot is not None:
            d.x_amax = self._slot_ptr(x.slot)
        if self.h2:
            assert x.slot is not None, name
            planes, sc2, winv = pk.h2()
            d.w_h2, d.scale_h2, d.winv_h2 = planes.data_ptr(), sc2.data_ptr(), winv.data_ptr()
        self.last_yslot = yslot
        y = None
        if segs is None:
            y = out if out is not None else self._new(x.B, Ho, Wo, pk.Cout)
            y.slot = yslot
            y.gain = og
            d.nseg = 1
            d.seg[0] = L.ConvSeg(0, pk.Cout, act, pk.Cout, Ho * Wo * pk.Cout, y.ptr)
        else:
            d.nseg = len(segs)
            for i, s in enumerate(segs):
                d.seg[i] = L.ConvSeg(*s)
        self.keepalive.append(pk)
        if not hasattr(self, '_desc_info'):
            self._desc_info = {}
        self._desc_info[C.addressof(d)] = (pk, res.slot if res is not None else None)
        wino = None
        if (self.use_winograd and dcn_offmask is None and out is None and pk.weight_oihw is not None and not wide
                and wino_eligible(pk, res, segs, act, x.C)):
            wino = [w for w in (self._wino_op(x, pk, act, y, name, segs, m) for m in self.wino_variants) if w is not None]
            wino = wino or None
        if dcn_offmask is not None:
            dd = L.DcnDesc()
            dd.conv = d
            dd.offmask, dd.ldo = dcn_offmask.ptr, dcn_offmask.C
            dd.om_layout = 1 if (self.om_pad and self.om_interleave) else 0
            self.ops.append((self.lib.ymi_dcn_v2_forward_f32, C.pointer(dd), name, self._cur))
            self.conv_meta.append((name, dd.conv))
            if wide:
                self.wide_ops.add(len(self.ops) - 1)
        else:
            self.ops.append((self.lib.ymi_conv2d_nhwc_f32, C.pointer(d), name, self._cur))
            self.conv_meta.append((name, d))
            if wide:
                self.wide_ops.add(len(self.ops) - 1)
            if wino is not None:
                self.wino_alt[len(self.ops) - 1] = wino
                if id(x) in self._upsrc:
                    self.wino_up[len(self.ops) - 1] = self._upsrc[id(x)]
        return y

    def _wino_op(self, x: T, pk: Packed, act, y: Optional[T], name, segs=None, m=2):
        key = (id(pk), m)
        wp = self._wino_packed.get(key)
        if wp is None:
            wp = self._wino_packed[key] = WinoPacked(pk.weight_oihw, self.device, m)
        th, tw = (x.H + m - 1) // m, (x.W + m - 1) // m
        Tn = x.B * th * tw
        Ng = _ceil(pk.Cout, 4)
        if Tn * max(pk.Cin, Ng) >= (1 << 29):
            return None
        g = (m + 2) * (m + 2)
        need_v, need_m = g * Tn * pk.Cin, g * Tn * Ng
        ws = self._wino_ws.setdefault(self._cur, [None, None])
        if ws[0] is None or ws[0].numel() < need_v:
            ws[0] = torch.empty(need_v, dtype=torch.float32, device=self.device)
        if ws[1] is None or ws[1].numel() < need_m:
            ws[1] = torch.empty(need_m, dtype=torch.float32, device=self.device)
        d = L.WinoDesc()
        d.x, d.u = x.ptr, wp.u.data_ptr()
        if self.split:
            d.u_x3 = wp.u3().data_ptr()
        if self.h2:
            planes, uinv = wp.h2()
            d.u_h2, d.uinv_h2 = planes.data_ptr(), uinv.data_ptr()
        if x.slot is not None:
            d.x_amax = self._slot_ptr(x.slot)
        if self.h2:
            d.y_amax = self._slot_ptr(self.last_yslot)
        if segs is None:
            d.y = y.ptr
        else:
            d.nseg = len(segs)
            for i, s in enumerate(segs):
                d.seg[i] = L.ConvSeg(*s)
        d.scale = pk.scale.data_ptr() if pk.scale is not None else None
        d.bias = pk.bias.data_ptr() if pk.bias is not None else None
        d.B, d.H, d.W, d.C, d.Cout, d.act, d.tile, d.m = x.B, x.H, x.W, pk.Cin, pk.Cout, act, L.TILE_AUTO, m
        d.cout_alg = pk.cout_alg
        return d

    def _bind_wino_workspaces(self):
        for idx, alts in self.wino_alt.items():
            ws = self._wino_ws[self.ops[idx][3]]
            for d in alts:
                d.V, d.M = ws[0].data_ptr(), ws[1].data_ptr()

    def call(self, fn, *args, name=''):
        self.ops.append((fn, args, name, self._cur))

    def _stage_done(self, li, t):
        sel = self.net.backbone_selected
        if not self._early_lat_on or li not in sel or sel.index(li) >= len(sel) - 1:
            return
        self._pending_lat.append((li, t))

    def _flush_early_laterals(self):
        sel = self.net.backbone_selected
        n = len(sel)
        for li, t in self._pending_lat:
            j = sel.index(li)
            i = n - 1 - j
            self.record('latgo%d' % i)
            self.on('B')
            self.wait('latgo%d' % i)
            raw = self.conv('fpn.lat%d' % i, t, self._pack(self.net.fpn.lat_layers[i]))
            self.record('lat%d' % i)
            self.on('A')
            self.early_lat[j] = raw
        self._pending_lat = []

    def on(self, which):
        self._cur = which if self.two_streams else 'A'

    def record(self, ev):
        if self.two_streams:
            self.events[ev] = torch.cuda.Event() if self.device.type == 'cuda' else None
            self.ops.append(('record', ev, ev, self._cur))

    def wait(self, ev):
        if self.two_streams:
            self.ops.append(('wait', ev, ev, self._cur))

    def _pack(self, conv, bn=None, cin_pad=None) -> Packed:
        key = (id(conv), id(bn), cin_pad)
        pk = self._pk_cache.get(key)
        if pk is None:
            pk = self._pk_cache[key] = pack_module(conv, bn, self.device, cin_pad)
        return pk

    def _rebalance_outliers(self, bb):
        self.rebalanced = []
        if not (self.h2 and os.environ.get('YOLACT_AMD_REBALANCE', '1') == '1' and isinstance(bb, M.ResNetBackbone)):
            return

        def exps(gain, cols, thr=6):
            g = gain.double().clamp_min(0)
            pos = g[g > 0]
            if pos.numel() < 8:
                return None
            kg = torch.floor(torch.log2((g / pos.median()).clamp_min(2.0 ** -126)))
            c = cols.double()
            cpos = c[c > 0]
            if cpos.numel() < 8:
                return None
            kc = torch.floor(torch.log2((cpos.median() / c.clamp_min(2.0 ** -126))))
            k = torch.minimum(kg, kc).clamp(min=0, max=40)
            k = torch.where((kg >= thr) & (kc >= thr) & (c > 0), k, torch.zeros_like(k))
            return k if bool((k > 0).any()) else None
        layers = list(bb.layers)
        sel = list(self.net.backbone_selected)
        fpn = self.net.fpn
        for li, layer in enumerate(layers):
            blocks = list(layer)
            if not blocks or blocks[0].downsample is None:
                continue
            prod = [self._pack(b.conv3, b.bn3) for b in blocks] + [self._pack(blocks[0].downsample[0], blocks[0].downsample[1])]
            cons = [self._pack(b.conv1, b.bn1) for b in blocks[1:]]
            if li + 1 < len(layers):
                nb = list(layers[li + 1])[0]
                cons.append(self._pack(nb.conv1, nb.bn1))
                if nb.downsample is not None:
                    cons.append(self._pack(nb.downsample[0], nb.downsample[1]))
            if li in sel:
                cons.append(self._pack(fpn.lat_layers[len(sel) - 1 - sel.index(li)]))
            if not cons or any(pk.Cin != prod[0].Cout or pk.Kpad != pk.kh * pk.kw * pk.Cin for pk in cons):
                continue
            gain = torch.stack([pk.out_gain()[:prod[0].Cout] for pk in prod]).amax(0)
            cols = torch.stack([pk.in_column_max() for pk in cons]).amax(0)
            k = exps(gain, cols)
            if k is None:
                continue
            down, up = torch.pow(2.0, -k).float(), torch.pow(2.0, k).float()
            for pk in prod:
                pk.scale_out_channels(down)
            for pk in cons:
                pk.scale_in_channels(up)
            self.rebalanced.append(('C%d' % (li + 2), int((k > 0).sum()), int(k.max())))
        pm_ = list(self.net.proto_net)
        self._proto0_down = None
        if (len(pm_) > 2 and isinstance(pm_[0], nn.Conv2d) and isinstance(pm_[1], nn.ReLU) and isinstance(pm_[2], nn.Conv2d)
                and pm_[0].bias is not None):
            p0, p2 = self._pack(pm_[0]), self._pack(pm_[2])
            if p2.Cin == p0.Cout and p2.Kpad == p2.kh * p2.kw * p2.Cin:
                k = exps(p0.out_gain(), p2.in_column_max())
                if k is not None:
                    down, up = torch.pow(2.0, -k).float(), torch.pow(2.0, k).float()
                    p0.scale_out_channels(down)
                    p2.scale_in_channels(up)
                    self._proto0_down = down
                    self.rebalanced.append(('proto_net.0', int((k > 0).sum()), int(k.max())))

    def _build(self):
        net, B, H, W, dev = self.net, self.B, self.H, self.W, self.device
        cfg = net.cfg
        lib = self.lib
        ar = self.arena

        self.early_lat, self._pending_lat = {}, []
        self._early_lat_on = self.two_streams and os.environ.get('YOLACT_AMD_EARLY_LAT', '0') == '1'
        bb = net.backbone
        self._pk_cache = {}
        self._rebalance_outliers(bb)
        c1 = getattr(bb, 'conv1', None)
        self.fused_stem = (self.h2 and isinstance(bb, M.ResNetBackbone) and os.environ.get('YOLACT_AMD_FUSED_STEM', '1') == '1'
                           and c1 is not None and tuple(c1.kernel_size) == (7, 7) and tuple(c1.stride) == (2, 2)
                           and tuple(c1.padding) == (3, 3) and c1.in_channels == 3 and c1.out_channels == 64 and H >= 7 and W >= 7)
        x4 = None
        if not self.fused_stem:
            x4 = self._new(B, H, W, 4, slot=self._slot())
            self.in_args = [None, x4.ptr, B, 3, H, W]
            self.in_amax = (x4.ptr, B * H * W * 4, self._slot_ptr(x4.slot))
            self.ops.append(('input', None, 'nchw_to_nhwc4', 'A'))
        if isinstance(bb, M.ResNetBackbone):
            outs = self._resnet(bb, x4)
        else:
            outs = self._darknet(bb, x4)
        self._flush_early_laterals()
        sel = [outs[i] for i in net.backbone_selected]
        for i, t in enumerate(outs):
            if i not in net.backbone_selected and t is not None:
                ar.free(t)

        fpn = net.fpn
        n = len(sel)
        sums = [None] * n
        prev = None
        for i in range(n):
            j = n - 1 - i
            pk = self._pack(fpn.lat_layers[i])
            if j in self.early_lat and prev is not None:
                raw = self.early_lat[j]
                self.wait('lat%d' % i)
                slot = self._slot()
                self.call(lib.ymi_bilinear_add_nhwc_f32, prev.ptr, raw.ptr, raw.B, prev.H, prev.W, raw.C, raw.H, raw.W,
                          self._slot_ptr(slot) if self.h2 else None, name='fpn.add%d' % i)
                raw.slot = slot
                if raw.gain is not None and prev.gain is not None and raw.gain.numel() == prev.gain.numel():
                    raw.gain = torch.maximum(raw.gain, prev.gain)
                sums[j] = raw
            elif prev is None:
                sums[j] = self.conv('fpn.lat%d' % i, sel[j], pk)
            else:
                sums[j] = self.conv('fpn.lat%d' % i, sel[j], pk, res=prev, res_mode=L.RES_BILINEAR)
            prev = sums[j]
        for t in sel:
            ar.free(t)

        shapes = [(t.H, t.W) for t in sums]
        for _ in fpn.downsample_layers:
            shapes.append((out_size(shapes[-1][0], 3, 2, 1), out_size(shapes[-1][1], 3, 2, 1)))
        self.feat_shapes = shapes
        nlev = len(shapes)

        pm = net.prediction_layers[0]
        A = pm.num_priors
        Ccls, D = cfg.num_classes, net.mask_dim
        cells = [h * w for h, w in shapes]
        P = sum(cells) * A
        self.P, self.A, self.D, self.Ccls = P, A, D, Ccls
        Cp = _ceil(Ccls, 4) if os.environ.get('YOLACT_AMD_PAD_CONF', '1') == '1' else Ccls
        self.conf_ld = Cp
        self.loc = torch.empty(B, P, 4, device=dev)
        self.conf = torch.zeros(B, P, Cp, device=dev)
        self.coef = torch.empty(B, P, D, device=dev)
        up_pk = [pack_module(m, device=dev) for m in pm.upfeature if isinstance(m, nn.Conv2d)] \
            if hasattr(pm, 'upfeature') else []
        cw, cb = pm.conf_layer.weight, pm.conf_layer.bias
        if Cp != Ccls:
            cw = torch.nn.functional.pad(cw.view(A, Ccls, *cw.shape[1:]), (0, 0, 0, 0, 0, 0, 0, Cp - Ccls)).reshape(A * Cp, *cw.shape[1:])
            cb = torch.nn.functional.pad(cb.view(A, Ccls), (0, Cp - Ccls)).reshape(A * Cp)
        wcat = torch.cat([pm.bbox_layer.weight, pm.mask_layer.weight, cw], 0)
        bcat = torch.cat([pm.bbox_layer.bias, pm.mask_layer.bias, cb], 0)
        hp = pm.bbox_layer
        head_pk = Packed(wcat, bcat, None, hp.stride[0], hp.padding[0], None, dev)
        head_pk.cout_alg = A * (4 + D + Ccls)
        coef_act = {'tanh': L.ACT_TANH, 'sigmoid': L.ACT_SIGMOID, 'relu': L.ACT_RELU, 'none': L.ACT_NONE}[
            act_name(cfg.mask_proto_coeff_activation)]
        n_b, n_c, n_m = A * 4, A * Cp, A * D
        offs = [sum(cells[:l]) * A for l in range(nlev)]
        bbc = cfg.backbone
        pri = []
        for lvl, (fh, fw) in enumerate(shapes):
            pri += make_priors_host(fh, fw, bbc.pred_scales[lvl], bbc.pred_aspect_ratios[lvl], cfg.max_size, bbc)

        pmods = list(net.proto_net)
        up_convs = [m for m in pm.upfeature if isinstance(m, nn.Conv2d)] if hasattr(pm, 'upfeature') else []
        self._merged_p3 = None
        merge_p3 = (os.environ.get('YOLACT_AMD_MERGE_P3', '1') == '1' and len(up_convs) == 1 and len(pmods) > 2
                    and isinstance(pmods[0], nn.Conv2d) and isinstance(pmods[1], nn.ReLU)
                    and all(c.kernel_size == (3, 3) and c.padding == (1, 1) and c.stride == (1, 1) and c.bias is not None
                            for c in (up_convs[0], pmods[0]))
                    and up_convs[0].in_channels == pmods[0].in_channels and up_convs[0].out_channels % 4 == 0
                    and pmods[0].out_channels % 4 == 0)

        def head(lvl, f):
            off = offs[lvl]
            u = f
            if lvl == 0 and merge_p3:
                cu, cp = up_convs[0], pmods[0]
                u = self._new(f.B, f.H, f.W, cu.out_channels)
                t0 = self._new(f.B, f.H, f.W, cp.out_channels)
                pkm = Packed(torch.cat([cu.weight, cp.weight], 0), torch.cat([cu.bias, cp.bias], 0), None, 1, 1, None, dev)
                if getattr(self, '_proto0_down', None) is not None:
                    pkm.scale_out_channels(torch.cat([torch.ones(cu.out_channels), self._proto0_down]))
                hw = f.H * f.W
                self.conv('head0.up0+proto.0', f, pkm, segs=[
                    (0, cu.out_channels, L.ACT_RELU, cu.out_channels, hw * cu.out_channels, u.ptr),
                    (cu.out_channels, cu.out_channels + cp.out_channels, L.ACT_RELU, cp.out_channels, hw * cp.out_channels,
                     t0.ptr)])
                u.slot, t0.slot = self.last_yslot, self.last_yslot + 1
                u.gain, t0.gain = self.last_out_gain[:cu.out_channels], self.last_out_gain[cu.out_channels:]
                self._merged_p3 = t0
            else:
                for k, pk in enumerate(up_pk):
                    nu = self.conv('head%d.up%d' % (lvl, k), u, pk, act=L.ACT_RELU)
                    if u is not f:
                        self.free(u)
                    u = nu
            segs = [
                (0, n_b, L.ACT_NONE, n_b, P * 4, self.loc.data_ptr() + off * 4 * 4),
                (n_b, n_b + n_m, coef_act, n_m, P * D, self.coef.data_ptr() + off * D * 4),
                (n_b + n_m, n_b + n_m + n_c, L.ACT_NONE, n_c, P * Cp, self.conf.data_ptr() + off * Cp * 4),
            ]
            self.conv('head%d.out' % lvl, u, head_pk, segs=segs)
            if u is not f:
                self.free(u)

        def pred(j):
            i = n - 1 - j
            return self.conv('fpn.pred%d' % i, sums[j], pack_module(fpn.pred_layers[i], device=dev), act=L.ACT_RELU)

        assert net.proto_src == 0, 'prototypes are taken from P3 in every shipped config'
        self.record('fork')
        self.on('B')
        self.wait('fork')
        self.on('A')
        p3 = pred(0)
        self.free(sums[0])
        self.on('B')
        feats_b = [pred(j) for j in range(1, n)]
        for j in range(1, n):
            self.free(sums[j])
        for i, m in enumerate(fpn.downsample_layers):
            feats_b.append(self.conv('fpn.down%d' % i, feats_b[-1], pack_module(m, device=dev)))
        self.on('A')
        head(0, p3)
        self.record('head0')
        self.on('B')
        for lvl in range(1, nlev):
            head(lvl, feats_b[lvl - 1])
        self.wait('head0')
        for f in feats_b:
            self.free(f)
        self.ops.append(('detect', None, 'detect', self._cur))
        self.record('b_done')
        self.on('A')

        t = p3
        mods = list(net.proto_net)
        conv_idx = [i for i, m in enumerate(mods) if isinstance(m, nn.Conv2d)]
        self.proto_patch = None
        self.proto_patch_wino = None
        self.wino_proj = None
        prev_conv_op = None
        held = None
        for i, m in enumerate(mods):
            if i == 0 and self._merged_p3 is not None:
                self.free(t)
                t = self._merged_p3
                continue
            if isinstance(m, nn.Conv2d):
                last = i == conv_idx[-1]
                has_relu = (i + 1 < len(mods) and isinstance(mods[i + 1], nn.ReLU))
                if last:
                    a = {'relu': L.ACT_RELU, 'none': L.ACT_NONE, 'sigmoid': L.ACT_SIGMOID, 'tanh': L.ACT_TANH}[
                        act_name(cfg.mask_proto_prototype_activation)]
                    assert not has_relu
                else:
                    a = L.ACT_RELU if has_relu else L.ACT_NONE
                pk = self._pack(m)
                if last:
                    Ho, Wo = out_size(t.H, pk.kh, pk.stride, pk.pad), out_size(t.W, pk.kw, pk.stride, pk.pad)
                    self.proto_shape = (B, Ho, Wo, pk.Cout)
                    self.conv('proto.%d' % i, t, pk, segs=[(0, pk.Cout, a, pk.Cout, Ho * Wo * pk.Cout, None)])
                    self.proto_patch = self.ops[-1][1].contents
                    nt = None
                    if (self.h2 and prev_conv_op is not None and prev_conv_op in self.wino_alt and (pk.kh, pk.kw, pk.stride, pk.pad) == (1, 1, 1, 0)
                            and pk.Cin == 256 and pk.Cout <= 32 and pk.Cout % 4 == 0 and a <= L.ACT_LEAKY01 and not getattr(pk, 'wide', False)
                            and os.environ.get('YOLACT_AMD_WINO_PROJ', '1') == '1'):
                        self.wino_proj = (prev_conv_op, len(self.ops) - 1)
                else:
                    nt = self.conv('proto.%d' % i, t, pk, act=a)
                    prev_conv_op = len(self.ops) - 1
                self.free(t)
                if held is not None:
                    self.free(held)
                    held = None
                t = nt
            elif isinstance(m, M.InterpolateModule):
                prev_conv_op = None
                s = int(m.scale_factor)
                has_relu = (i + 1 < len(mods) and isinstance(mods[i + 1], nn.ReLU))
                y = self._new(t.B, t.H * s, t.W * s, t.C, slot=t.slot, gain=t.gain)
                self.call(lib.ymi_bilinear_nhwc_f32, t.ptr, y.ptr, t.B, t.H, t.W, t.C, y.H, y.W,
                          C.c_float(1.0 / s), C.c_float(1.0 / s), 1 if has_relu else 0, name='proto.interp')
                if s == 2 and os.environ.get('YOLACT_AMD_FUSED_UPSAMPLE', '1') == '1':
                    self._upsrc[id(y)] = (len(self.ops) - 1, t.ptr, 1 if has_relu else 0)
                    held = t
                else:
                    self.free(t)
                t = y
        assert self.proto_patch is not None and held is None
        self.wait('b_done')
        self.priors = torch.tensor(pri, dtype=torch.float32).view(-1, 4).to(dev)
        assert self.priors.shape[0] == P

    def _resnet(self, bb: M.ResNetBackbone, x4: T):
        dev, ar, lib = self.device, self.arena, self.lib
        pk0 = pack_module(bb.conv1, bb.bn1, dev, cin_pad=4)
        if self.fused_stem:
            B, H, W = self.B, self.H, self.W
            Hs, Ws = out_size(H, 7, 2, 3), out_size(W, 7, 2, 3)
            Hp, Wp = out_size(Hs, 3, 2, 1), out_size(Ws, 3, 2, 1)
            x = self._new(B, Hp, Wp, 64, slot=self._slot(), gain=pk0.out_gain())
            planes, sc2, winv = pk0.h2()
            sd = L.StemDesc()
            sd.y, sd.B, sd.H, sd.W, sd.cout_pad, sd.kpad = x.ptr, B, H, W, pk0.CoutPad, pk0.Kpad
            sd.w_h2, sd.scale_h2, sd.bias, sd.y_amax = planes.data_ptr(), sc2.data_ptr(), pk0.bias.data_ptr(), self._slot_ptr(x.slot)
            self.keepalive.append(pk0)
            md = L.ConvDesc()
            md.B, md.H, md.W, md.Cin, md.ldx, md.Ho, md.Wo, md.Cout = B, H, W, 4, 4, Hs, Ws, 64
            md.kh, md.kw, md.stride, md.pad, md.Kpad, md.cin_alg, md.cout_alg = 7, 7, 2, 3, pk0.Kpad, 3, 64
            self.conv_meta.append(('stem', md))
            self.ops.append(('stem', sd, 'stem+maxpool', 'A'))
            self._stem_desc = sd
        else:
            stem = self.conv('stem', x4, pk0, act=L.ACT_RELU)
            ar.free(x4)
            Hp, Wp = out_size(stem.H, 3, 2, 1), out_size(stem.W, 3, 2, 1)
            x = self._new(stem.B, Hp, Wp, stem.C, slot=stem.slot, gain=stem.gain)
            self.call(lib.ymi_maxpool3x3s2_nhwc_f32, stem.ptr, x.ptr, stem.B, stem.H, stem.W, stem.C, Hp, Wp, name='maxpool')
            ar.free(stem)
        outs = []
        self._stage_out_ptr = {}
        held = []
        for li, layer in enumerate(bb.layers):
            for bi, blk in enumerate(layer):
                nm = 'layer%d.%d' % (li, bi)
                side_down = blk.downsample is not None and self.two_streams and self.down_on_side_stream
                if side_down:
                    self.record(nm + '.in')
                    self.on('B')
                    self.wait(nm + '.in')
                    res = self.conv(nm + '.down', x, self._pack(blk.downsample[0], blk.downsample[1]))
                    self.record(nm + '.down')
                    self.on('A')
                o1 = self.conv(nm + '.conv1', x, self._pack(blk.conv1, blk.bn1), act=L.ACT_RELU)
                for t in held:
                    ar.free(t)
                held = []
                if blk.use_dcn:
                    dcn = blk.conv2
                    om = self.conv(nm + '.offmask', o1, pack_offmask(dcn.conv_offset_mask, dev, self.om_interleave) if self.om_pad
                                   else pack_module(dcn.conv_offset_mask, None, dev))
                    pk = Packed(dcn.weight, dcn.bias, blk.bn2, dcn.stride[0], 1, None, dev)
                    o2 = self.conv(nm + '.dcn', o1, pk, act=L.ACT_RELU, dcn_offmask=om)
                    ar.free(om)
                else:
                    o2 = self.conv(nm + '.conv2', o1, pack_module(blk.conv2, blk.bn2, dev), act=L.ACT_RELU)
                ar.free(o1)
                if side_down:
                    self.wait(nm + '.down')
                elif blk.downsample is not None:
                    res = self.conv(nm + '.down', x, self._pack(blk.downsample[0], blk.downsample[1]))
                else:
                    res = x
                y = self.conv(nm + '.conv3', o2, self._pack(blk.conv3, blk.bn3), act=L.ACT_RELU, res=res,
                              res_mode=L.RES_ADD)
                hold = (self.h2 and bi == len(layer) - 1 and li + 1 < len(bb.layers) and blk.downsample is None
                        and o2.C == 64 and y.C == 256)
                if hold:
                    held = [o2, x]
                else:
                    ar.free(o2)
                if side_down:
                    self.on('B')
                    self.free(res)
                    self.on('A')
                elif res is not x:
                    ar.free(res)
                if not hold:
                    ar.free(x)
                x = y
                if bi == 0:
                    self._flush_early_laterals()
            outs.append(x)
            self._stage_out_ptr[li] = x.ptr
            self._stage_done(li, x)
            x = _Borrowed(x)
        for t in held:
            ar.free(t)
        return outs

# ... 237 lines not shown
```

### yolact_amd/plan_tune.py

```python
from __future__ import annotations

import ctypes as C
import os

import torch

from . import _lib as L
from . import tune_table as TT


def _ceil(a, b):
    return (a + b - 1) // b * b


def _desc_pointers(d):
    out = []
    if isinstance(d, C.Array):
        for e in d:
            out += _desc_pointers(e) if isinstance(e, (C.Structure, C.Array)) else ([int(e)] if isinstance(e, int) and e else [])
        return out
    for f in d._fields_:
        name, typ = f[0], f[1]
        v = getattr(d, name)
        if typ is C.c_void_p:
            if v:
                out.append(int(v))
        elif isinstance(v, (C.Structure, C.Array)) and (issubclass(typ, C.Structure) or issubclass(getattr(typ, '_type_', int), (C.Structure, C.c_void_p))):
            out += _desc_pointers(v)
    return out


def _split_k_ids(tid, blocks, nk, Cout):
    out = []
    if blocks < 400 and Cout % 4 == 0:
        for S in (2, 3, 4, 5, 6, 8, 9, 12, 16):
            per = -(-nk // S)
            if per >= 4 and per * (S - 1) < nk and 128 <= blocks * S <= 1100:
                out.append(TT.direct_choice(tid, S))
    return out


def _timed(run, e0, e1, reps):
    run()
    best = 1e30
    for _ in range(2):
        e0.record()
        for _ in range(reps):
            run()
        e1.record()
        e1.synchronize()
        best = min(best, e0.elapsed_time(e1) / reps)
    return best


def _rows_overlap(M, a, lda, b, ldb):
    a, b = int(a or 0), int(b or 0)
    return a < b + 4 * M * int(ldb) and b < a + 4 * M * int(lda)


def _fill_chain(cd, d3, d1=None):
    cd.x, cd.res, cd.y = d3.x, d3.res, d3.seg[0].ptr
    cd.w_a_h2, cd.scale_a_h2, cd.bias_a = d3.w_h2, d3.scale_h2, d3.bias
    cd.x_amax, cd.y_amax = d3.x_amax, d3.y_amax
    cd.M, cd.ldx, cd.res_ld, cd.ldy = d3.B * d3.Ho * d3.Wo, d3.ldx, d3.res_ld, d3.seg[0].row_stride
    cd.k_a, cd.n_a, cd.n_b = d3.Cin, d3.Cout, d1.Cout if d1 is not None else d3.Cin
    cd.cout_pad_a, cd.cout_pad_b = _ceil(cd.n_a, 128), _ceil(cd.n_b, 128)
    cd.act_a = d3.seg[0].act
    if d1 is not None:
        cd.z, cd.ldz, cd.z_amax, cd.act_b = d1.seg[0].ptr, d1.seg[0].row_stride, d1.y_amax, d1.seg[0].act
        cd.w_b_h2, cd.scale_b_h2, cd.bias_b = d1.w_h2, d1.scale_h2, d1.bias
    return cd


def _set_wino_choice(wd, v):
    wd.tile, wd.v_planes = TT.wino_parts(v)


class PlanTuning:
    def tune(self, x: torch.Tensor, reps: int = 3):
        mode = os.environ.get('YOLACT_AMD_AUTOTUNE', '1')
        self.tune_table, self.wino_table, self.tune_misses = [], [], 0
        if mode == '0':
            return []
        cache_path = os.environ.get('YOLACT_AMD_TUNE_CACHE')
        disk = {}
        if mode != 'force':
            disk.update(TT.load_tune_table(self.device))
            if cache_path and os.path.exists(cache_path):
                disk.update(TT.read_table_file(cache_path))
        n0 = len(disk)
        self.run(x)
        s = L.stream_ptr()
        e0, e1 = torch.cuda.Event(enable_timing=True), torch.cuda.Event(enable_timing=True)
        measure = mode != 'table'
        self._tune_direct(e0, e1, s, reps, disk, measure)
        self._tune_winograd(e0, e1, s, reps, disk, measure)
        self._fuse_pointwise_chains(e0, e1, s, reps, disk, measure)
        torch.cuda.synchronize(self.device)
        if cache_path and (len(disk) != n0 or mode == 'force'):
            TT.write_table_file(cache_path, disk, self.device)
        self.tune_entries = disk
        return self.tune_table

    def _splitk_ws(self, where, numel):
        ws = self._sk_ws.get(where)
        if ws is None or ws.numel() < numel:
            ws = self._sk_ws[where] = torch.empty(numel, dtype=torch.float32, device=self.device)
            for fn, dptr, _n, w in self.ops:
                if fn is self.lib.ymi_conv2d_nhwc_f32 and w == where and dptr.contents.split_k > 1:
                    dptr.contents.split_ws = ws.data_ptr()
                elif fn is self.lib.ymi_dcn_v2_forward_f32 and w == where and dptr.contents.conv.split_k > 1:
                    dptr.contents.conv.split_ws = ws.data_ptr()
        return ws

    @staticmethod
    def _splitk_ok(d):
        return (d.kh == 1 and d.kw == 1 and d.pad == 0 and d.Cin == d.Kpad and d.Cin % 32 == 0 and d.nseg == 1
                and d.Cout % 4 == 0 and d.seg[0].act <= L.ACT_LEAKY01 and d.res_mode in (L.RES_NONE, L.RES_ADD)
                and d.B * d.Ho * d.Wo <= 16384 and d.Kpad >= 256)

    def _fuse_pointwise_chains(self, e0, e1, s, reps, disk, measure):
        self.chain_table, self.chainx_table, self.chaine_table = [], [], []
        if not self.h2 or os.environ.get('YOLACT_AMD_CHAIN', '1') != '1':
            return
        lib = self.lib

        def timed(run):
            return _timed(run, e0, e1, reps)
        entry_mode = os.environ.get('YOLACT_AMD_CHAIN_ENTRY', '1')
        entry = {i3: idn for idn, i3, _ in self.entry_chain_candidates()} if entry_mode in ('1', 'force') else {}
        self._fuse_stage_exit(s, disk, measure, timed)
        i = 0
        while i < len(self.ops):
            f3, p3, n3, w3 = self.ops[i]
            i += 1
            if f3 is not lib.ymi_conv2d_nhwc_f32 or (i - 1) in self.wide_ops:
                continue
            d3 = p3.contents
            M = d3.B * d3.Ho * d3.Wo
            P_ = d3.Cin
            if not ((d3.kh, d3.kw, d3.stride, d3.pad, d3.nseg) == (1, 1, 1, 0, 1) and P_ in (64, 128, 256) and d3.Cout == 4 * P_
                    and d3.res_mode == L.RES_ADD and not d3.res_after_act and d3.seg[0].n0 == 0 and d3.seg[0].act <= L.ACT_LEAKY01
                    and d3.w_h2 and d3.x_amax and M * max(d3.seg[0].row_stride, d3.res_ld) < (1 << 29)):
                continue
            if P_ > 64 and os.environ.get('YOLACT_AMD_CHAIN2', '0') not in ('1', 'force'):
                continue
            pair = False
            if i < len(self.ops) and self.ops[i][0] is lib.ymi_conv2d_nhwc_f32 and self.ops[i][3] == w3 and i not in self.wide_ops:
                d1 = self.ops[i][1].contents
                pair = ((d1.kh, d1.kw, d1.stride, d1.pad, d1.Cin, d1.Cout, d1.nseg) == (1, 1, 1, 0, 4 * P_, P_, 1)
                        and d1.res_mode == L.RES_NONE and d1.x == d3.seg[0].ptr and d1.ldx == d3.seg[0].row_stride
                        and d1.seg[0].n0 == 0 and d1.seg[0].act <= L.ACT_LEAKY01 and bool(d1.w_h2))
            if P_ > 64 and not pair:
                continue
            cd = _fill_chain(L.ChainDesc(), d3, d1 if pair else None)
            if P_ > 64:
                info = getattr(self, '_desc_info', {}).get(C.addressof(d3))
                if info is None or info[1] is None:
                    continue
                cd.gain_a, cd.bias_max_a = info[0].l1_gain()
                cd.res_amax = self._slot_ptr(info[1])
            name = n3
            if pair:
                f1, p1, n1, w1 = self.ops[i]
                name = n3 + '+' + n1
                in_place = int(cd.z) == int(cd.x) and cd.ldz == cd.ldx
                if (_rows_overlap(M, cd.z, cd.ldz, cd.y, cd.ldy) or _rows_overlap(M, cd.z, cd.ldz, cd.res, cd.res_ld)
                        or (_rows_overlap(M, cd.z, cd.ldz, cd.x, cd.ldx) and not in_place)):
                    continue
            cptr = C.pointer(cd)
            key = TT.chain_key('chain' if pair else 'chain1', d3.B, d3.Ho, d3.Wo, P_ if P_ > 64 else None, self.mode)
            ent = disk.get(key)
            if P_ > 64 and os.environ.get('YOLACT_AMD_CHAIN2') == 'force':
                ent = [1, 0.0, 0.0]
            if ent is None:
                self.tune_misses += 1
                if not measure or lib.ymi_pointwise_chain_f32(cptr, s) != 0:
                    continue
                t_plan = timed((lambda: (f3(p3, s), f1(p1, s))) if pair else (lambda: f3(p3, s)))
                t_one = timed(lambda: lib.ymi_pointwise_chain_f32(cptr, s))
                ent = disk[key] = [1 if t_one < 0.97 * t_plan else 0, round(t_plan, 4), round(t_one, 4)]
            self.chain_table.append((name, ent[0], ent[1], ent[2]))
            if ent[0] and lib.ymi_pointwise_chain_f32(cptr, s) == 0:
                self.keepalive.append(cd)
                self.ops[i - 1] = (lib.ymi_pointwise_chain_f32, cptr, name, w3)
                if pair:
                    self.ops[i] = ('nop', None, n1 + '[fused into ' + n3 + ']', w1)
                    i += 1
                    if P_ == 64 and (i - 2) in entry:
                        self._fuse_entry_shortcut(i - 2, entry[i - 2], cd, s, disk, measure, timed, entry_mode)

    def _fuse_entry_shortcut(self, ic, idn, cd, s, disk, measure, timed, mode):
        lib = self.lib
        fd, pd, nd, wd = self.ops[idn]
        ce = self._entry_chain_desc(cd, idn)
        if ce is None:
            return
        dd = pd.contents
        eptr, cptr = C.pointer(ce), C.pointer(cd)
        key = TT.chain_key('chain', dd.B, dd.Ho, dd.Wo, 64, self.mode)
        ent = disk.get(key)
        if mode == 'force':
            ent = [1, 0.0, 0.0]
        if ent is None:
            self.tune_misses += 1
            if not measure or lib.ymi_pointwise_chain_f32(eptr, s) != 0:
                return
            t_plan = timed(lambda: (fd(pd, s), lib.ymi_pointwise_chain_f32(cptr, s)))
            t_one = timed(lambda: lib.ymi_pointwise_chain_f32(eptr, s))
            ent = disk[key] = [1 if t_one < 0.97 * t_plan else 0, round(t_plan, 4), round(t_one, 4)]
        fc, _, nc, wc = self.ops[ic]
        self.chaine_table.append((nc, ent[0], ent[1], ent[2]))
        if ent[0] and lib.ymi_pointwise_chain_f32(eptr, s) == 0:
            self.keepalive.append(ce)
            self.ops[ic] = (fc, eptr, nc, wc)
            self.ops[idn] = ('nop', None, nd + '[fused into ' + nc.split('+')[0] + ']', wd)
            names = [n for n, _ in self.conv_meta]
            n3 = nc.split('+')[0]
            if nd in names and n3 in names:
                m = self.conv_meta.pop(names.index(nd))
                self.conv_meta.insert([n for n, _ in self.conv_meta].index(n3) + 1, m)

    def stage_exit_candidates(self):
        conv = self.lib.ymi_conv2d_nhwc_f32
        selected = {int(p) for li, p in getattr(self, '_stage_out_ptr', {}).items() if li in self.net.backbone_selected}
        out = []
        for i3, (f3, p3, n3, w3) in enumerate(self.ops):
            if f3 is not conv or i3 in self.wide_ops:
                continue
            d3 = p3.contents
            if not ((d3.kh, d3.kw, d3.stride, d3.pad, d3.nseg, d3.Cin, d3.Cout) == (1, 1, 1, 0, 1, 64, 256)
                    and d3.res_mode == L.RES_ADD and not d3.res_after_act and d3.seg[0].n0 == 0 and d3.seg[0].act <= L.ACT_LEAKY01):
                continue
            yptr, ldy = int(d3.seg[0].ptr or 0), d3.seg[0].row_stride
            if not yptr or yptr in selected:
                continue
            i1 = None
            for j in range(i3 + 1, len(self.ops)):
                fj, pj, _, wj = self.ops[j]
                if wj != w3 or fj in ('record', 'nop'):
                    continue
                if fj is conv and j not in self.wide_ops:
                    d1 = pj.contents
                    if ((d1.kh, d1.kw, d1.stride, d1.pad, d1.Cin, d1.Cout, d1.nseg) == (1, 1, 1, 0, 256, 128, 1)
                            and d1.res_mode == L.RES_NONE and int(d1.x or 0) == yptr and d1.ldx == ldy
                            and (d1.B, d1.H, d1.W) == (d3.B, d3.Ho, d3.Wo) and d1.seg[0].n0 == 0 and d1.seg[0].act <= L.ACT_LEAKY01):
                        i1 = j
                break
            if i1 is None:
# ... 187 lines not shown
    def patch2_candidates(d):
        if os.environ.get('YOLACT_AMD_PATCH2', '1') != '1':
            return []
        if not ((d.kh, d.kw, d.stride, d.pad) == (3, 3, 1, 1) and d.Cin % 32 == 0 and d.Kpad == 9 * d.Cin and d.Cout >= 64 and d.Cout % 4 == 0
                and d.res_mode == L.RES_NONE and 1 <= d.nseg <= 3 and d.w_h2):
            return []
        cov = 0
        for i in range(d.nseg):
            g = d.seg[i]
            if (g.n0 != cov or g.n0 % 128 or g.act > L.ACT_LEAKY01 or g.act < 0 or g.row_stride % 4 or g.row_stride < g.n1 - g.n0
                    or g.batch_stride != d.Ho * d.Wo * g.row_stride):
                return []
            cov = g.n1
        if cov < d.Cout:
            return []
        return [t | L.TILE_H2 | L.TILE_DCNP for t in sorted(L.PATCH2_TILES)]

    @staticmethod
    def pc_candidates(d):
        if os.environ.get('YOLACT_AMD_PC', '0') != '1' or d.Cout <= 32:
            return []
        M, nk = d.B * d.Ho * d.Wo, d.Kpad // 32
        out = []
        for t, name in sorted(L.PC_TILES.items()):
            bm, bn = (int(v) for v in os.environ.get('YOLACT_AMD_PC_SHAPE', name[2:]).split('x'))
            if bn > 128 and d.Cout < 256:
                continue
            tid = t | L.TILE_H2 | L.TILE_DCNP
            out.append(tid)
            out += _split_k_ids(tid, -(-M // bm) * -(-d.Cout // bn), nk, d.Cout)
        return out

    @staticmethod
    def ws_candidates(d):
        if d.res_mode != L.RES_NONE or d.Cout > 64:
            return []
        M, nk = d.B * d.Ho * d.Wo, d.Kpad // 32
        out = []
        for t, name in sorted(L.WS_TILES.items()):
            bm, bn = (int(v) for v in name[2:].split('w')[0].split('x'))
            if (bn == 32) != (d.Cout <= 32):
                continue
            cap = (64 * 1024) // (bn * 128)
            blocks, n = -(-M // bm), 0
            for S in (1, 2, 3, 4, 5, 6, 8, 9, 12, 16):
                per = -(-nk // S)
                if per > cap or (S > 1 and per * (S - 1) >= nk):
                    continue
                if n and blocks * S > 1200:
                    break
                out.append(TT.direct_choice(t | L.TILE_H2 | L.TILE_DCNP, S))
                n += 1
                if n == 3:
                    break
        return out

    def direct_key(self, fn, d, wide=False):
        is_dcn = fn is self.lib.ymi_dcn_v2_forward_f32
        h2_, split_ = self.h2 and not wide, self.split or (wide and not is_dcn)
        return TT.desc_key(d, 'x3' if split_ else 'h2' if h2_ else '', dcn=is_dcn)

    def direct_candidates(self, fn, d, wide=False):
        is_dcn = fn is self.lib.ymi_dcn_v2_forward_f32
        h2_, split_ = self.h2 and not wide, self.split or (wide and not is_dcn)
        if is_dcn:
            cands = [t for t in L.BASIC_TILES if t != L.TILE_128x32]
        elif d.Cin % 32 != 0:
            cands = [L.TILE_128x64, L.TILE_64x64] if d.Cout <= 64 else list(L.BASIC_TILES)
        elif d.Cout <= 32:
            cands = [L.TILE_128x32, L.TILE_64x64, L.TILE_64x64_S3, L.TILE_32x32_K4, L.TILE_32x32_K4_S4,
                     L.TILE_64x32_K2, L.TILE_64x32_K2_S3]
        elif d.Cout <= 64:
            cands = [L.TILE_128x64, L.TILE_128x64_S3, L.TILE_64x64, L.TILE_64x64_S3, L.TILE_64x64_S4,
                     L.TILE_32x32_K4, L.TILE_32x32_K4_S4, L.TILE_64x32_K2, L.TILE_64x32_K2_S3,
                     L.TILE_32x64_K2, L.TILE_32x64_K2_S3]
        else:
            cands = [t for t in sorted(L.TILE_NAMES) if t != L.TILE_128x32 and not (t & (L.TILE_X3 | L.TILE_H2))]
            if d.Cout < 256:
                cands = [t for t in cands if t != L.TILE_128x256_W8]
        spflag = (L.TILE_X3 if split_ else L.TILE_H2 if h2_ else 0) if not (is_dcn and split_) else 0
        if spflag:
            base_ok = L.H2_BASE_TILES if spflag == L.TILE_H2 else L.X3_BASE_TILES
            cands = cands + [t | spflag for t in cands if t in base_ok
                             and (d.Cin % 32 == 0 or t in L.BASIC_TILES)]
        if is_dcn and h2_:
            cands = cands + self.dcnp_candidates(d, dcn=True)
        if not is_dcn and h2_ and self.pipe and self._pipe_ok(d):
            cands = cands + self.dcnp_candidates(d) + self.ws_candidates(d)
            cands = cands + self.pc_candidates(d)
        if not is_dcn and h2_ and self.pipe:
            cands = cands + self.patch2_candidates(d)
            if ((d.kh, d.kw, d.stride, d.pad, d.Cin, d.Cout) == (3, 3, 1, 1, 64, 64) and d.res_mode == L.RES_NONE
                    and TT.patch_tile_allowed()):
                cands = cands + [L.DCNP_PATCH_C64 | L.TILE_H2 | L.TILE_DCNP]
        if not is_dcn and self._splitk_ok(d) and self.splitk:
            x3 = spflag
            for S in (2, 4):
                if (d.Kpad // 32) % S == 0 and d.Kpad // S >= 128:
                    cands += [TT.direct_choice(t | x3, S) for t in (L.TILE_128x128, L.TILE_64x128, L.TILE_128x64, L.TILE_64x64,
                                                                    L.TILE_256x128_W8)]

        return cands

    def _tune_direct(self, e0, e1, s, reps, disk, measure):
        cache = {}
        cname = TT.choice_name
        for opi, (fn, dptr, name, where) in enumerate(self.ops):
            is_dcn = fn is self.lib.ymi_dcn_v2_forward_f32
            if fn is not self.lib.ymi_conv2d_nhwc_f32 and not is_dcn:
                continue
            d = dptr.contents.conv if is_dcn else dptr.contents
            wide = opi in self.wide_ops
            skey = self.direct_key(fn, d, wide)
            key = (skey, wide)
            if key not in cache and skey in disk:
                v_ = int(disk[skey])
                patch_off = (TT.direct_parts(v_)[0] == (L.DCNP_PATCH_C64 | L.TILE_H2 | L.TILE_DCNP) and not TT.patch_tile_allowed())
                if not patch_off and self._apply_choice(fn, dptr, where, disk[skey], s) == 0:
                    cache[key] = v_
            if key not in cache:
                self.tune_misses += 1
                if not measure:
                    cache[key] = L.TILE_AUTO
                    d.tile, d.split_k = L.TILE_AUTO, 0
                    continue
                cands = self.direct_candidates(fn, d, wide)
                best, best_ms, times = None, 1e30, {}
                ok_cands = []
                for t in cands:
                    if self._apply_choice(fn, dptr, where, t, s) == 0:
                        ok_cands.append(t)
                yslot = self.amax[(d.y_amax - self.amax.data_ptr()) // 4:][:L.AMAX_SLOT_FLOATS] if d.y_amax else None
                for rnd in range(2):
                    for t in ok_cands:
                        self._apply_choice(fn, dptr, where, t, s)
                        e0.record()
                        for _ in range(reps):
                            if yslot is not None:
                                yslot.zero_()
                            fn(dptr, s)
                        e1.record()
                        e1.synchronize()
                        ms = e0.elapsed_time(e1) / reps
                        times[cname(t)] = round(min(ms, times.get(cname(t), 1e30)), 4)
                for t in ok_cands:
                    if times[cname(t)] < best_ms:
                        best, best_ms = t, times[cname(t)]
                assert best is not None, name
                cache[key] = best
                disk[skey] = best
                self.tune_table.append((name, cname(best), times))
            self._apply_choice(fn, dptr, where, cache[key], s)

    def _tune_winograd(self, e0, e1, s, reps, disk, measure):
        lib = self.lib
        self.wino_toggle = {}
        wtiles = [L.TILE_64x64, L.TILE_64x128, L.TILE_128x64, L.TILE_128x128_W8, L.TILE_64x128_S3, L.TILE_32x64_K2,
                  L.TILE_128x128, L.TILE_128x128_S3, L.TILE_128x128_W8_S3, L.TILE_256x128_W8, L.TILE_256x128_W8_S3]
        if self.split:
            wtiles = wtiles + [t | L.TILE_X3 for t in wtiles]
        if self.h2:
            hb = wtiles + [L.TILE_128x256_W8]
            wtiles = wtiles + [t | L.TILE_H2 for t in hb] + [TT.wino_choice(t | L.TILE_H2, planes=1) for t in hb]
            if os.environ.get('YOLACT_AMD_WGEMM', '1') == '1':
                wtiles = wtiles + [TT.wino_choice(L.TILE_WG_128x256 | L.TILE_H2, planes=1)]
        memo = {}
        for idx, alts in sorted(self.wino_alt.items()):
            fn, dptr, name, where = self.ops[idx]
            if fn is not lib.ymi_conv2d_nhwc_f32:
                continue
            w0 = alts[0]
            key = TT.wino_key(w0.B, w0.H, w0.W, w0.C, w0.Cout, w0.act, w0.nseg, tuple(a.m for a in alts), self.mode)
            if key not in memo and key in disk:
                ent = tuple(disk[key])
                ok = True
                if ent[1]:
                    wd = [a for a in alts if a.m == ent[0]]
                    if wd:
                        _set_wino_choice(wd[0], ent[1])
                        ok = lib.ymi_conv3x3_winograd_f32(C.byref(wd[0]), s) == 0
                    else:
                        ok = False
                if ok:
                    memo[key] = ent
            if key not in memo:
                self.tune_misses += 1
                if not measure:
                    memo[key] = (0, 0, 0.0, 0.0, 0.0, 0.0)
                else:
                    t_direct = _timed(lambda: fn(dptr, s), e0, e1, reps)
                    best_m, best_t, best_ms, per_m = 0, 0, 1e30, {}
                    for wd in alts:
                        for t in wtiles:
                            _set_wino_choice(wd, t)
                            if lib.ymi_conv3x3_winograd_f32(C.byref(wd), s) != 0:
                                continue
                            wptr = C.pointer(wd)
                            ms = _timed(lambda: lib.ymi_conv3x3_winograd_f32(wptr, s), e0, e1, reps)
                            per_m[wd.m] = min(ms, per_m.get(wd.m, 1e30))
                            if ms < best_ms:
                                best_m, best_t, best_ms = wd.m, t, ms
                    memo[key] = (best_m, best_t, round(t_direct, 4), round(best_ms, 4),
                                 round(per_m.get(2, 0.0), 4), round(per_m.get(4, 0.0), 4))
                    disk[key] = list(memo[key])
            best_m, best_t, t_direct, t_wino, t_f2, t_f4 = memo[key]
            best_tile, best_planes = TT.wino_parts(best_t)
            self.wino_table.append((name, 'F%d/%s%s' % (best_m, L.TILE_NAMES.get(best_tile, '-'), 'p' if best_planes else ''),
                                    t_direct, t_wino, t_f2, t_f4))
            instep_direct = disk.get(TT.instep_key(key)) == 0 and not self.wino_force
            if best_t and not (self.wino_up.get(idx) is not None or (self.wino_proj is not None and self.wino_proj[0] == idx)):
                wd_ = [a for a in alts if a.m == best_m][0]
                _set_wino_choice(wd_, best_t)
                self.wino_toggle.setdefault(key, []).append(
                    (idx, (fn, dptr, name, where), (lib.ymi_conv3x3_winograd_f32, C.pointer(wd_), name + '[wino]', where),
                     bool(t_wino < 0.97 * t_direct)))
            if best_t and (self.wino_force or (t_wino < 0.97 * t_direct and not instep_direct)):
                wd = [a for a in alts if a.m == best_m][0]
                _set_wino_choice(wd, best_t)
                self.ops[idx] = (lib.ymi_conv3x3_winograd_f32, C.pointer(wd), name + '[wino]', where)
                up = self.wino_up.get(idx)
                if up is not None and best_m == 4 and wd.H % 2 == 0 and wd.W % 2 == 0:
                    bidx, lo_ptr, relu = up
                    wd.x_up, wd.up_relu = lo_ptr, relu
                    bfn, bargs, bname, bwhere = self.ops[bidx]
                    self.ops[bidx] = ('nop', None, bname + '[fused into ' + name + ']', bwhere)
                if self.wino_proj is not None and self.wino_proj[0] == idx and best_m == 4 and wd.Cout == 256 and wd.nseg == 0:
                    pidx = self.wino_proj[1]
                    pfn, pdptr, pname, pwhere = self.ops[pidx]
                    if pfn is lib.ymi_conv2d_nhwc_f32 and pwhere == where:
                        pd = pdptr.contents
                        wd.proj_w_h2, wd.proj_scale_h2, wd.proj_bias = pd.w_h2, pd.scale_h2, pd.bias
                        wd.proj_y, wd.proj_y_amax = pd.seg[0].ptr, pd.y_amax
                        wd.proj_cout, wd.proj_ldy, wd.proj_act = pd.Cout, pd.seg[0].row_stride, pd.seg[0].act
                        scratch = torch.empty(self.proto_shape, dtype=torch.float32, device=self.device)
                        wd.proj_y = scratch.data_ptr()
                        rc = lib.ymi_conv3x3_winograd_f32(C.byref(wd), s)
                        torch.cuda.synchronize(self.device)
                        wd.proj_y = None
                        if rc != 0:
                            wd.proj_w_h2 = None
                            self.wino_proj_rejected = rc
                        else:
                            self.ops[pidx] = ('nop', None, pname + '[fused into ' + name + ']', pwhere)
                            self.proto_patch_wino = wd

    def set_winograd(self, key, on: bool):
        for idx, direct_op, wino_op, _ in self.wino_toggle.get(key, []):
            self.ops[idx] = wino_op if on else direct_op
```

### yolact_amd/tune_table.py

```python
import ast
import json
import os
import re

from . import _lib as L

TUNE_GEN = 5
TUNE_DIR = os.path.join(os.path.dirname(os.path.abspath(__file__)), 'tune')
_table_cache = {}


def read_table_file(path):
    try:
        with open(path) as f:
            doc = json.load(f)
    except (OSError, ValueError):
        return {}
    if not isinstance(doc, dict) or doc.get('gen') != TUNE_GEN or not isinstance(doc.get('abi'), int) or doc['abi'] > L.ABI_VERSION:
        return {}
    return dict(doc.get('entries', {}))


def write_table_file(path, entries, device=None, note=None):
    name = None
    if device is not None and device.type == 'cuda':
        import torch
        name = torch.cuda.get_device_name(device)
    doc = {'gen': TUNE_GEN, 'abi': L.ABI_VERSION, 'device': name,
           'note': note or 'tile id per conv shape (B,H,W,Cin,Cout,kh,kw,stride,pad,res_mode,nseg,Kpad); wino(...) -> '
                           '[m, gemm tile, direct ms, winograd ms, F(2x2) ms, F(4x4) ms]',
           'entries': {k: entries[k] for k in sorted(entries)}}
    tmp = path + '.tmp%d' % os.getpid()
    with open(tmp, 'w') as f:
        json.dump(doc, f, indent=0, separators=(',', ':'))
    os.replace(tmp, path)


def load_tune_table(device):
    arch = 'gfx950'
    if device.type == 'cuda':
        import torch
        arch = getattr(torch.cuda.get_device_properties(device), 'gcnArchName', 'gfx950').split(':')[0]
    if arch not in _table_cache:
        _table_cache[arch] = read_table_file(os.path.join(TUNE_DIR, arch + '.json'))
    return dict(_table_cache[arch])


def build_meta():
    try:
        with open(os.path.join(os.path.dirname(os.path.abspath(__file__)), 'build_meta.json')) as f:
            doc = json.load(f)
        return doc if isinstance(doc, dict) else {}
    except (OSError, ValueError):
        return {}


def patch_tile_allowed():
    return os.environ.get('YOLACT_AMD_PATCH', '1') == '1' and build_meta().get('lint', 'ok') != 'skipped'


MODES = ('', 'h2', 'x3')
KINDS = ('conv', 'dcn', 'wino', 'chain', 'chain1', 'chainx', 'instep')
_PREFIX = {'conv': '', 'dcn': '', 'wino': 'wino', 'chain': 'chain', 'chain1': 'chain1', 'chainx': 'chainx'}
_INSTEP = 'instep|'
_KEY_RE = re.compile(r'(instep\|)?(wino|chain1|chainx|chain|)(\(.*\))(?:\|(h2|x3))?')


def _ints(t, n):
    return len(t) in n and all(type(v) is int for v in t)


def _valid(kind, t):
    if type(t) is not tuple:
        return False
    if kind == 'conv':
        return _ints(t, (12,))
    if kind == 'dcn':
        return len(t) == 13 and _ints(t[:12], (12,)) and t[12] == 'dcn'
    if kind == 'wino':
        return len(t) == 8 and _ints(t[:7], (7,)) and type(t[7]) is tuple and _ints(t[7], (1, 2))
    return _ints(t, (3,) if kind == 'chainx' else (3, 4))


def format(kind, t, mode=''):
    t = tuple(t)
    inner = 'wino' if kind == 'instep' else kind
    if inner not in _PREFIX or mode not in MODES or not _valid(inner, t):
        raise ValueError('no tune-table key: %r' % ((kind, t, mode),))
    return (_INSTEP if kind == 'instep' else '') + _PREFIX[inner] + str(t) + ('|' + mode if mode else '')


def parse(key):
    m = _KEY_RE.fullmatch(key) if isinstance(key, str) else None
    try:
        instep, head, t, mode = m.group(1), m.group(2), ast.literal_eval(m.group(3)), m.group(4) or ''
        kind = head or ('dcn' if len(t) == 13 else 'conv')
        if instep:
            kind = {'wino': 'instep'}[kind]
        if format(kind, t, mode) == key:
            return kind, t, mode
    except (AttributeError, KeyError, TypeError, ValueError, SyntaxError, MemoryError, RecursionError):
        pass
    raise ValueError('no tune-table key: %r' % (key,))


def conv_key(shape, mode='', dcn=False):
    return format('dcn', tuple(shape) + ('dcn',), mode) if dcn else format('conv', shape, mode)


def desc_key(d, mode='', dcn=False):
    return conv_key((d.B, d.H, d.W, d.Cin, d.Cout, d.kh, d.kw, d.stride, d.pad, d.res_mode, d.nseg, d.Kpad), mode, dcn)


def wino_key(B, H, W, C, Cout, act, nseg, ms, mode=''):
    return format('wino', (B, H, W, C, Cout, act, nseg, tuple(ms)), mode)


def chain_key(kind, B, H, W, P=None, mode=''):
    if kind not in ('chain', 'chain1'):
        raise ValueError(kind)
    return format(kind, (B, H, W) + ((P,) if P is not None else ()), mode)


def chainx_key(B, H, W, mode=''):
    return format('chainx', (B, H, W), mode)


def instep_key(wino):
    kind, t, mode = parse(wino)
    if kind != 'wino':
        raise ValueError('no wino key: %r' % (wino,))
    return format('instep', t, mode)


def direct_choice(tile, split_k=0):
    return int(tile) + 256 * (int(split_k) if split_k > 1 else 0)


def direct_parts(v):
    return int(v) & 255, int(v) >> 8


def wino_choice(tile, planes=0):
    return int(tile) | (L.WINO_PLANES if planes else 0)


def wino_parts(v):
    return int(v) & 255, 1 if int(v) & L.WINO_PLANES else 0


def choice_name(v):
    tile, S = direct_parts(v)
    return L.TILE_NAMES.get(tile, '?%d' % tile) + ('/k%d' % S if S else '')
```

Measured before the change: 2403.

## Merge per-level prediction-head Winograd convs across FPN levels into one launch

```diff
diff --git a/include/yolact_amd.h b/include/yolact_amd.h
--- a/include/yolact_amd.h
+++ b/include/yolact_amd.h
@@ -111,6 +111,16 @@
   const float *proj_scale_h2, *proj_bias;
   float *proj_y, *proj_y_amax;
   int32_t proj_cout, proj_ldy, proj_act, _pad5;
+  int32_t nlev, nabs;
+  struct {
+    const float *x;
+    const float *x_amax;
+    float *y, *y_amax;
+    int64_t seg_off[3];
+    int32_t H, W;
+  } lev[5];
+  float *lev_amax;
+  double abs_flops[8];
 } ymi_wino_desc;
 int ymi_conv3x3_winograd_f32(const ymi_wino_desc *d, void *stream);
 
diff --git a/yolact_amd/_lib.py b/yolact_amd/_lib.py
--- a/yolact_amd/_lib.py
+++ b/yolact_amd/_lib.py
@@ -76,6 +76,11 @@
                 ('y_amax', C.c_void_p), ('x_amax_mul', C.c_float), ('_pad3', C.c_int32)]
 
 
+class WinoLevel(C.Structure):
+    _fields_ = [('x', C.c_void_p), ('x_amax', C.c_void_p), ('y', C.c_void_p), ('y_amax', C.c_void_p),
+                ('seg_off', C.c_int64 * 3), ('H', C.c_int32), ('W', C.c_int32)]
+
+
 class WinoDesc(C.Structure):
     _fields_ = [('x', C.c_void_p), ('u', C.c_void_p), ('scale', C.c_void_p), ('bias', C.c_void_p), ('y', C.c_void_p),
                 ('V', C.c_void_p), ('M', C.c_void_p),
@@ -86,7 +91,9 @@
                 ('x_up', C.c_void_p), ('up_relu', C.c_int32), ('_pad4', C.c_int32),
                 ('proj_w_h2', C.c_void_p), ('proj_scale_h2', C.c_void_p), ('proj_bias', C.c_void_p),
                 ('proj_y', C.c_void_p), ('proj_y_amax', C.c_void_p),
-                ('proj_cout', C.c_int32), ('proj_ldy', C.c_int32), ('proj_act', C.c_int32), ('_pad5', C.c_int32)]
+                ('proj_cout', C.c_int32), ('proj_ldy', C.c_int32), ('proj_act', C.c_int32), ('_pad5', C.c_int32),
+                ('nlev', C.c_int32), ('nabs', C.c_int32), ('lev', WinoLevel * 5), ('lev_amax', C.c_void_p),
+                ('abs_flops', C.c_double * 8)]
 
 
 class DcnDesc(C.Structure):
diff --git a/yolact_amd/csrc/api.cpp b/yolact_amd/csrc/api.cpp
--- a/yolact_amd/csrc/api.cpp
+++ b/yolact_amd/csrc/api.cpp
@@ -45,8 +45,17 @@
     case YMI_WS_WINO_M: {
       const ymi_wino_desc *d = (const ymi_wino_desc *)desc;
       const int m = d->m == 4 ? 4 : 2;
+      int64_t G = (int64_t)(m + 2) * (m + 2), T = 0;
+      if (d->nlev != 0) {
+        if (d->nlev < 2 || d->nlev > 5 || d->m != 4 || d->B < 1 || d->C < 1 || d->Cout < 1) return -1;
+        for (int l = 0; l < d->nlev; ++l) {
+          if (d->lev[l].H < 1 || d->lev[l].W < 1) return -1;
+          T += (int64_t)d->B * cdiv(d->lev[l].H, 4) * cdiv(d->lev[l].W, 4);
+        }
+        return 4 * G * T * (what == YMI_WS_WINO_V ? (int64_t)d->C : cdiv(d->Cout, 4) * 4);
+      }
       if ((d->m != 0 && d->m != 2 && d->m != 4) || d->B < 1 || d->H < 1 || d->W < 1 || d->C < 1 || d->Cout < 1) return -1;
-      const int64_t G = (int64_t)(m + 2) * (m + 2), T = (int64_t)d->B * cdiv(d->H, m) * cdiv(d->W, m);
+      T = (int64_t)d->B * cdiv(d->H, m) * cdiv(d->W, m);
       return 4 * G * T * (what == YMI_WS_WINO_V ? (int64_t)d->C : cdiv(d->Cout, 4) * 4);
     }
     case YMI_WS_SPLITK: {
diff --git a/yolact_amd/csrc/winograd.hip b/yolact_amd/csrc/winograd.hip
--- a/yolact_amd/csrc/winograd.hip
+++ b/yolact_amd/csrc/winograd.hip
@@ -285,15 +285,65 @@
   l1 = src - (float)i0;
 }
 
-template <bool PLANES, bool UPS = false>
+struct NoLev {};
+struct LevTab {
+  int nlev;
+  int t0[5];
+  int H[5], W[5], th[5], tw[5];
+  const float *x[5];
+  const float *x_amax[5];
+  float *y[5], *y_amax[5];
+  long off[5][3];
+  float *pub;
+};
+struct LevGeo { int l, H, W, th, tw; unsigned t0; };
+__device__ __forceinline__ LevGeo lev_pick(const LevTab &lt, unsigned tu) {
+  LevGeo g = {0, lt.H[0], lt.W[0], lt.th[0], lt.tw[0], 0u};
+#pragma unroll
+  for (int k = 1; k < 5; ++k)
+    if (k < lt.nlev && tu >= (unsigned)lt.t0[k]) { g.l = k; g.H = lt.H[k]; g.W = lt.W[k]; g.th = lt.th[k]; g.tw = lt.tw[k]; g.t0 = (unsigned)lt.t0[k]; }
+  return g;
+}
+template <class P>
+__device__ __forceinline__ P lev_sel(P const (&a)[5], int l) {
+  P v = a[0];
+#pragma unroll
+  for (int k = 1; k < 5; ++k) v = l == k ? a[k] : v;
+  return v;
+}
+__device__ __forceinline__ float lev_amax_read(const LevTab &lt) {
+  float m = ymi_amax_read(lt.x_amax[0]);
+#pragma unroll
+  for (int k = 1; k < 5; ++k)
+    if (k < lt.nlev) m = fmaxf(m, ymi_amax_read(lt.x_amax[k]));
+  return m;
+}
+
+template <bool PLANES, bool UPS = false, class LT = NoLev>
 __global__ __launch_bounds__(256) void wino43_in_k(const float *__restrict__ x, float *__restrict__ V, int H, int W, int C4,
                                                    int th, int tw, long T, long total, const float *__restrict__ x_amax,
-                                                   int up_relu = 0) {
+                                                   int up_relu, const LT lt) {
+  constexpr bool LEV = !__is_same(LT, NoLev);
   float vs = 1.f, vinv = 1.f;
-  if (PLANES) ymi_h2_scale(ymi_amax_read(x_amax) * 100.f, vs, vinv);
+  if constexpr (LEV) {
+    if (PLANES || lt.pub) {
+      const float bound = lev_amax_read(lt);
+      if (PLANES) ymi_h2_scale(bound * 100.f, vs, vinv);
+      if (lt.pub && blockIdx.x == 0 && threadIdx.x == 0) lt.pub[0] = bound;
+    }
+  } else {
+    if (PLANES) ymi_h2_scale(ymi_amax_read(x_amax) * 100.f, vs, vinv);
+  }
   for (unsigned i = blockIdx.x * 256u + threadIdx.x; i < (unsigned)total; i += gridDim.x * 256u) {
-    const unsigned tu = i / (unsigned)C4, ru = tu / (unsigned)tw, bu = ru / (unsigned)th;
-    const int c4 = (int)(i - tu * (unsigned)C4), tx = (int)(tu - ru * (unsigned)tw), ty = (int)(ru - bu * (unsigned)th);
+    const unsigned tu = i / (unsigned)C4;
+    unsigned tl = tu;
+    if constexpr (LEV) {
+      const LevGeo g = lev_pick(lt, tu);
+      H = g.H; W = g.W; th = g.th; tw = g.tw; tl = tu - g.t0;
+      x = lev_sel(lt.x, g.l);
+    }
+    const unsigned ru = tl / (unsigned)tw, bu = ru / (unsigned)th;
+    const int c4 = (int)(i - tu * (unsigned)C4), tx = (int)(tl - ru * (unsigned)tw), ty = (int)(ru - bu * (unsigned)th);
     const long t = tu, b = bu;
     const int y0 = 4 * ty - 1, x0 = 4 * tx - 1;
     f32x4 u[6][6];
@@ -389,15 +439,33 @@
   for (int iy = 0; iy < 4; ++iy) at6(s[iy][0], s[iy][1], s[iy][2], s[iy][3], s[iy][4], s[iy][5], o[iy][0], o[iy][1], o[iy][2], o[iy][3]);
 }
 
+__device__ __forceinline__ void lev_amax_add(float (&am)[5], int l, float v) {
+#pragma unroll
+  for (int k = 0; k < 5; ++k) am[k] = l == k ? fmaxf(am[k], v) : am[k];
+}
+
+template <class LT = NoLev>
 __global__ __launch_bounds__(256) void wino43_out_k(const float *__restrict__ Mm, float *__restrict__ y,
                                                     const float *__restrict__ scale, const float *__restrict__ bias, int Ho,
                                                     int Wo, int N4, int th, int tw, long T, int act, long total,
-                                                    float *__restrict__ y_amax) {
+                                                    float *__restrict__ y_amax, const LT lt) {
+  constexpr bool LEV = !__is_same(LT, NoLev);
   float am = 0.f;
-  const ymi_amax_pre apre = ymi_amax_prefetch(y_amax);
+  float aml[5] = {0.f, 0.f, 0.f, 0.f, 0.f};
+  ymi_amax_pre apre;
+  if constexpr (!LEV) apre = ymi_amax_prefetch(y_amax);
   for (unsigned i = blockIdx.x * 256u + threadIdx.x; i < (unsigned)total; i += gridDim.x * 256u) {
-    const unsigned tu = i / (unsigned)N4, ru = tu / (unsigned)tw, bu = ru / (unsigned)th;
-    const int n4 = (int)(i - tu * (unsigned)N4), tx = (int)(tu - ru * (unsigned)tw), ty = (int)(ru - bu * (unsigned)th);
+    const unsigned tu = i / (unsigned)N4;
+    unsigned tl = tu;
+    int lv = 0;
+    if constexpr (LEV) {
+      const LevGeo g = lev_pick(lt, tu);
+      Ho = g.H; Wo = g.W; th = g.th; tw = g.tw; tl = tu - g.t0; lv = g.l;
+      y = lev_sel(lt.y, g.l);
+      am = 0.f;
+    }
+    const unsigned ru = tl / (unsigned)tw, bu = ru / (unsigned)th;
+    const int n4 = (int)(i - tu * (unsigned)N4), tx = (int)(tl - ru * (unsigned)tw), ty = (int)(ru - bu * (unsigned)th);
     const long t = tu, b = bu;
     f32x4 o[4][4];
     wino43_out_tile(Mm + t * (N4 * 4L) + n4 * 4, T * (N4 * 4L), o);
@@ -423,8 +491,15 @@
         const int oy = 4 * ty + iy, ox = 4 * tx + ix;
         if (oy < Ho && ox < Wo) *reinterpret_cast<f32x4 *>(y + ((b * Ho + oy) * (long)Wo + ox) * (N4 * 4L) + n4 * 4) = o[iy][ix];
       }
-  }
-  if (y_amax) ymi_amax_finish(apre, am);
+    if constexpr (LEV) lev_amax_add(aml, lv, am);
+  }
+  if constexpr (LEV) {
+#pragma unroll
+    for (int k = 0; k < 5; ++k)
+      if (k < lt.nlev && lt.y_amax[k]) ymi_amax_finish(ymi_amax_prefetch(lt.y_amax[k]), aml[k]);
+  } else {
+    if (y_amax) ymi_amax_finish(apre, am);
+  }
 }
 
 struct ProjArgs {
@@ -531,14 +606,33 @@
 #endif
 }
 
-__global__ __launch_bounds__(256) void wino43_out_seg_k(const float *__restrict__ Mm, const SegTab st,
+template <class LT = NoLev>
+__global__ __launch_bounds__(256) void wino43_out_seg_k(const float *__restrict__ Mm, const SegTab st0,
                                                         const float *__restrict__ scale, const float *__restrict__ bias,
-                                                        int Ho, int Wo, int N4, int Cout, int th, int tw, long T, long total, float *__restrict__ y_amax) {
+                                                        int Ho, int Wo, int N4, int Cout, int th, int tw, long T, long total,
+                                                        float *__restrict__ y_amax, const LT lt) {
+  constexpr bool LEV = !__is_same(LT, NoLev);
   float am[3] = {0.f, 0.f, 0.f};
   const ymi_amax_pre apre = ymi_amax_prefetch(y_amax);
   for (unsigned i = blockIdx.x * 256u + threadIdx.x; i < (unsigned)total; i += gridDim.x * 256u) {
-    const unsigned tu = i / (unsigned)N4, ru = tu / (unsigned)tw, bu = ru / (unsigned)th;
-    const int n4 = (int)(i - tu * (unsigned)N4), tx = (int)(tu - ru * (unsigned)tw), ty = (int)(ru - bu * (unsigned)th);
+    const unsigned tu = i / (unsigned)N4;
+    unsigned tl = tu;
+    SegTab stl;
+    if constexpr (LEV) {
+      const LevGeo g = lev_pick(lt, tu);
+      Ho = g.H; Wo = g.W; th = g.th; tw = g.tw; tl = tu - g.t0;
+      stl = st0;
+#pragma unroll
+      for (int k = 0; k < 3; ++k) {
+        long off = lt.off[0][k];
+#pragma unroll
+        for (int q = 1; q < 5; ++q) off = g.l == q ? lt.off[q][k] : off;
+        stl.seg[k].ptr = st0.seg[k].ptr ? st0.seg[k].ptr + off : nullptr;
+      }
+    }
+    const SegTab &st = LEV ? stl : st0;
+    const unsigned ru = tl / (unsigned)tw, bu = ru / (unsigned)th;
+    const int n4 = (int)(i - tu * (unsigned)N4), tx = (int)(tl - ru * (unsigned)tw), ty = (int)(ru - bu * (unsigned)th);
     const long t = tu, b = bu;
     f32x4 o[4][4];
     wino43_out_tile(Mm + t * (N4 * 4L) + n4 * 4, T * (N4 * 4L), o);
@@ -581,7 +675,7 @@
       }
     }
   }
-  seg_amax_commit(y_amax, st.nseg, apre, am);
+  seg_amax_commit(y_amax, st0.nseg, apre, am);
 }
 
 unsigned grid_for(long total) {
@@ -592,7 +686,90 @@
 
 }
 
+static int wino_levels(const ymi_wino_desc *d, hipStream_t s) {
+  if (d->nlev < 2 || d->nlev > 5 || d->m != 4 || !(d->tile & YMI_TILE_H2) || (d->tile & YMI_TILE_X3) || d->x_up || d->proj_w_h2 ||
+      (d->v_planes != 0 && d->v_planes != 1) || d->nabs < 0 || d->nabs > 8)
+    return YMI_EARG;
+  if (d->B <= 0 || d->C <= 0 || d->Cout <= 0 || d->nseg < 0 || d->nseg > 3) return YMI_EARG;
+  LevTab lt = {};
+  lt.nlev = d->nlev;
+  long T = 0;
+  bool one_slot = true;
+  for (int l = 0; l < d->nlev; ++l) {
+    if (d->lev[l].H <= 0 || d->lev[l].W <= 0) return YMI_EARG;
+    for (int k = 0; k < d->nseg; ++k) if (d->lev[l].seg_off[k] & 3) return YMI_EARG;
+    if (!d->lev[l].x || !d->lev[l].x_amax || (d->nseg == 0 && !d->lev[l].y)) return YMI_ENULL;
+    lt.H[l] = d->lev[l].H; lt.W[l] = d->lev[l].W;
+    lt.th[l] = (d->lev[l].H + 3) / 4; lt.tw[l] = (d->lev[l].W + 3) / 4;
+    lt.x[l] = d->lev[l].x; lt.x_amax[l] = d->lev[l].x_amax; lt.y[l] = d->lev[l].y; lt.y_amax[l] = d->lev[l].y_amax;
+    for (int k = 0; k < 3; ++k) lt.off[l][k] = (long)(d->lev[l].seg_off[k] / 4);
+    one_slot = one_slot && d->lev[l].x_amax == d->lev[0].x_amax;
+    if (T >= (1L << 29)) return YMI_ESHAPE;
+    lt.t0[l] = (int)T;
+    T += (long)d->B * lt.th[l] * lt.tw[l];
+  }
+  if (!d->u || !d->V || !d->M || !d->u_h2 || !d->uinv_h2 || (!one_slot && !d->lev_amax)) return YMI_ENULL;
+  if (d->nseg == 0 && ((d->Cout & 3) || d->act > YMI_ACT_LEAKY01 || d->act < 0)) return YMI_ESHAPE;
+  for (int k = 0; k < d->nseg; ++k) if (!d->seg[k].ptr) return YMI_ENULL;
+  if (d->C & 31) return YMI_ESHAPE;
+  const int Ng = (d->Cout + 3) / 4 * 4;
+  if (T * (long)(d->C > Ng ? d->C : Ng) >= (1L << 29)) return YMI_ESHAPE;
+  const int C4 = d->C / 4, N4 = Ng / 4;
+  const float *bound = one_slot ? d->lev[0].x_amax : d->lev_amax;
+  lt.pub = one_slot ? nullptr : d->lev_amax;
+  const bool planes = d->v_planes != 0;
+  if ((d->tile & 31) == YMI_TILE_WG_128x256 && !planes) return YMI_EARG;
+  const double alg = 2.0 * d->B * d->lev[0].H * d->lev[0].W * (double)(d->cout_alg > 0 ? d->cout_alg : d->Cout) * 9.0 * d->C;
+  const double exe = 2.0 * 36 * (double)T * d->C * Ng;
+  const int outer = ymi_internal_prof_begin(alg, d->tile, 4, s);
+  const float *nox = nullptr;
+  if (planes) hipLaunchKernelGGL((wino43_in_k<true, false, LevTab>), dim3(grid_for(T * C4)), dim3(256), 0, s, nox, d->V, 0, 0, C4, 0, 0, T, T * C4, nox, 0, lt);
+  else hipLaunchKernelGGL((wino43_in_k<false, false, LevTab>), dim3(grid_for(T * C4)), dim3(256), 0, s, nox, d->V, 0, 0, C4, 0, 0, T, T * C4, nox, 0, lt);
+  int rc = ymi_launch_status();
+  if (rc) return rc;
+  const long cout_pad = ((long)d->Cout + 127) / 128 * 128;
+  if ((d->tile & 31) == YMI_TILE_WG_128x256) {
+    rc = ymi_internal_wgemm(d->V, d->u_h2, d->uinv_h2, bound, 100.f, d->M, 36, T, d->C, Ng, (int)cout_pad, exe, 6, s);
+  } else {
+    ymi_conv_desc g = {};
+    g.x = d->V; g.w = d->u;
+    g.B = 1; g.H = (int)T; g.W = 1; g.Cin = d->C; g.ldx = d->C;
+    g.Ho = (int)T; g.Wo = 1; g.Cout = Ng;
+    g.kh = g.kw = 1; g.stride = 1; g.pad = 0; g.Kpad = d->C;
+    g.nseg = 1; g.tile = d->tile;
+    g.w_h2 = d->u_h2; g.scale_h2 = d->uinv_h2; g.winv_h2 = d->uinv_h2;
+    g.x_amax = bound; g.x_amax_mul = 100.f;
+    g.seg[0].n0 = 0; g.seg[0].n1 = Ng; g.seg[0].act = YMI_ACT_NONE; g.seg[0].row_stride = Ng;
+    g.seg[0].batch_stride = T * Ng; g.seg[0].ptr = d->M;
+    if (planes)
+      rc = ymi_internal_grouped_gemm(&g, 36, T * d->C, cout_pad * d->C, T * Ng, exe, 6, s, d->V, (unsigned)(T * d->C * 2),
+                                     2L * T * d->C * 2, (unsigned)cout_pad);
+    else
+      rc = ymi_internal_grouped_gemm(&g, 36, T * d->C, cout_pad * d->C, T * Ng, exe, 6, s, nullptr, 0, 0, (unsigned)cout_pad);
+  }
+  if (rc) return rc;
+  if (d->nseg > 0) {
+    SegTab st;
+    st.nseg = d->nseg;
+    for (int k = 0; k < 3; ++k) st.seg[k] = d->seg[k];
+    hipLaunchKernelGGL(wino43_out_seg_k<LevTab>, dim3(grid_for(T * N4)), dim3(256), 0, s, d->M, st, d->scale, d->bias, 0, 0, N4, d->Cout,
+                       0, 0, T, T * N4, d->y_amax, lt);
+  } else {
+    float *noy = nullptr;
+    hipLaunchKernelGGL(wino43_out_k<LevTab>, dim3(grid_for(T * N4)), dim3(256), 0, s, d->M, noy, d->scale, d->bias, 0, 0, N4, 0, 0, T,
+                       d->act, T * N4, noy, lt);
+  }
+  rc = ymi_launch_status();
+  ymi_internal_prof_end(outer, s);
+  for (int i = 0; rc == YMI_OK && i < d->nabs; ++i) {
+    const int pr = ymi_internal_prof_begin(d->abs_flops[i], d->tile, 12, s);
+    ymi_internal_prof_end(pr, s);
+  }
+  return rc;
+}
+
 extern "C" int ymi_conv3x3_winograd_f32(const ymi_wino_desc *d, void *stream) {
+  if (d && d->nlev != 0) return wino_levels(d, (hipStream_t)stream);
   if (!d || (!d->x && !d->x_up) || !d->u || !d->V || !d->M) return YMI_ENULL;
   if (d->x_up && (d->m != 4 || (d->H & 1) || (d->W & 1) || (((uintptr_t)d->x_up) & 15))) return YMI_ESHAPE;
   if (d->B <= 0 || d->H <= 0 || d->W <= 0 || d->C <= 0 || d->Cout <= 0 || d->nseg < 0 || d->nseg > 3) return YMI_EARG;
@@ -625,10 +802,10 @@
 #endif
   if (mt == 4) {
     if (d->x_up) {
-      if (planes) hipLaunchKernelGGL((wino43_in_k<true, true>), dim3(grid_for(T * C4)), dim3(256), 0, s, d->x_up, d->V, d->H, d->W, C4, th, tw, T, T * C4, d->x_amax, d->up_relu);
-      else hipLaunchKernelGGL((wino43_in_k<false, true>), dim3(grid_for(T * C4)), dim3(256), 0, s, d->x_up, d->V, d->H, d->W, C4, th, tw, T, T * C4, d->x_amax, d->up_relu);
-    } else if (planes) hipLaunchKernelGGL((wino43_in_k<true, false>), dim3(grid_for(T * C4)), dim3(256), 0, s, d->x, d->V, d->H, d->W, C4, th, tw, T, T * C4, d->x_amax, 0);
-    else hipLaunchKernelGGL((wino43_in_k<false, false>), dim3(grid_for(T * C4)), dim3(256), 0, s, d->x, d->V, d->H, d->W, C4, th, tw, T, T * C4, d->x_amax, 0);
+      if (planes) hipLaunchKernelGGL((wino43_in_k<true, true>), dim3(grid_for(T * C4)), dim3(256), 0, s, d->x_up, d->V, d->H, d->W, C4, th, tw, T, T * C4, d->x_amax, d->up_relu, NoLev{});
+      else hipLaunchKernelGGL((wino43_in_k<false, true>), dim3(grid_for(T * C4)), dim3(256), 0, s, d->x_up, d->V, d->H, d->W, C4, th, tw, T, T * C4, d->x_amax, d->up_relu, NoLev{});
+    } else if (planes) hipLaunchKernelGGL((wino43_in_k<true, false>), dim3(grid_for(T * C4)), dim3(256), 0, s, d->x, d->V, d->H, d->W, C4, th, tw, T, T * C4, d->x_amax, 0, NoLev{});
+    else hipLaunchKernelGGL((wino43_in_k<false, false>), dim3(grid_for(T * C4)), dim3(256), 0, s, d->x, d->V, d->H, d->W, C4, th, tw, T, T * C4, d->x_amax, 0, NoLev{});
   } else {
     if (planes) hipLaunchKernelGGL(wino_in_k<true>, dim3(grid_for(T * C4)), dim3(256), 0, s, d->x, d->V, d->H, d->W, C4, th, tw, T, T * C4, d->x_amax);
     else hipLaunchKernelGGL(wino_in_k<false>, dim3(grid_for(T * C4)), dim3(256), 0, s, d->x, d->V, d->H, d->W, C4, th, tw, T, T * C4, d->x_amax);
@@ -666,8 +843,8 @@
     st.nseg = d->nseg;
     for (int k = 0; k < 3; ++k) st.seg[k] = d->seg[k];
     if (mt == 4)
-      hipLaunchKernelGGL(wino43_out_seg_k, dim3(grid_for(T * N4)), dim3(256), 0, s, d->M, st, d->scale, d->bias, d->H, d->W,
-                         N4, d->Cout, th, tw, T, T * N4, d->y_amax);
+      hipLaunchKernelGGL(wino43_out_seg_k<NoLev>, dim3(grid_for(T * N4)), dim3(256), 0, s, d->M, st, d->scale, d->bias, d->H, d->W,
+                         N4, d->Cout, th, tw, T, T * N4, d->y_amax, NoLev{});
     else
       hipLaunchKernelGGL(wino_out_seg_k, dim3(grid_for(T * N4)), dim3(256), 0, s, d->M, st, d->scale, d->bias, d->H, d->W, N4,
                          d->Cout, th, tw, T, T * N4, d->y_amax);
@@ -691,8 +868,8 @@
     return rc;
   }
   if (mt == 4)
-    hipLaunchKernelGGL(wino43_out_k, dim3(grid_for(T * N4)), dim3(256), 0, s, d->M, d->y, d->scale, d->bias, d->H, d->W, N4, th,
-                       tw, T, d->act, T * N4, d->y_amax);
+    hipLaunchKernelGGL(wino43_out_k<NoLev>, dim3(grid_for(T * N4)), dim3(256), 0, s, d->M, d->y, d->scale, d->bias, d->H, d->W, N4, th,
+                       tw, T, d->act, T * N4, d->y_amax, NoLev{});
   else
     hipLaunchKernelGGL(wino_out_k, dim3(grid_for(T * N4)), dim3(256), 0, s, d->M, d->y, d->scale, d->bias, d->H, d->W, N4, th,
                        tw, T, d->act, T * N4, d->y_amax);
diff --git a/yolact_amd/engine.py b/yolact_amd/engine.py
--- a/yolact_amd/engine.py
+++ b/yolact_amd/engine.py
@@ -371,6 +371,7 @@
         self._sk_ws = {}
         self.down_on_side_stream = os.environ.get('YOLACT_AMD_DOWN_STREAM', 'B') == 'B'
         self.wino_alt, self._wino_packed, self._wino_ws = {}, {}, {}
+        self.level_merge, self.merged_levels = None, False
         self._upsrc, self.wino_up = {}, {}
         self._done_event = None
         self._priors_timed = False
@@ -538,6 +539,81 @@
             ws = self._wino_ws[self.ops[idx][3]]
             for d in alts:
                 d.V, d.M = ws[0].data_ptr(), ws[1].data_ptr()
+        if self.level_merge is not None:
+            ws = self._wino_ws[self.level_merge['where']]
+            for d in self.level_merge['descs']:
+                d.V, d.M = ws[0].data_ptr(), ws[1].data_ptr()
+
+    def _build_level_merge(self, lev_ops, up_pk, head_pk, offs, widths, ncols, coef_act):
+        self.level_merge = None
+        self.merged_levels = False
+        lv = sorted(l for l in lev_ops if l >= 1)
+        if not (self.h2 and 2 <= len(lv) <= 5 and len(up_pk) == 1 and all(len(lev_ops[l]) == 3 for l in lv)):
+            return
+        pku = up_pk[0]
+        if not all((pk.kh, pk.kw, pk.stride, pk.pad) == (3, 3, 1, 1) and pk.weight_oihw is not None and pk.Cin % 32 == 0
+                   and not getattr(pk, 'wide', False) for pk in (pku, head_pk)) or pku.Cout % 32 != 0:
+            return
+        if any(i in self.wide_ops for l in lv for i in lev_ops[l][1:]):
+            return
+        feats = [lev_ops[l][0] for l in lv]
+        B = feats[0].B
+        Tn = sum(B * _ceil(f.H, 4) // 4 * (_ceil(f.W, 4) // 4) for f in feats)
+        if Tn * max(pku.Cin, pku.Cout, _ceil(head_pk.Cout, 4)) >= (1 << 29):
+            return
+        ws = self._wino_ws.setdefault(self._cur, [None, None])
+        need_v, need_m = 36 * Tn * max(pku.Cin, pku.Cout), 36 * Tn * max(pku.Cout, _ceil(head_pk.Cout, 4))
+        if ws[0] is None or ws[0].numel() < need_v:
+            ws[0] = torch.empty(need_v, dtype=torch.float32, device=self.device)
+        if ws[1] is None or ws[1].numel() < need_m:
+            ws[1] = torch.empty(need_m, dtype=torch.float32, device=self.device)
+        mid = [torch.empty(B * f.H * f.W * pku.Cout, dtype=torch.float32, device=self.device) for f in feats]
+        uslot, pubslot = self._slot(), self._slot()
+
+        def base(pk, act):
+            key = (id(pk), 4)
+            wp = self._wino_packed.get(key)
+            if wp is None:
+                wp = self._wino_packed[key] = WinoPacked(pk.weight_oihw, self.device, 4)
+            d = L.WinoDesc()
+            d.u = wp.u.data_ptr()
+            planes, uinv = wp.h2()
+            d.u_h2, d.uinv_h2 = planes.data_ptr(), uinv.data_ptr()
+            d.scale = pk.scale.data_ptr() if pk.scale is not None else None
+            d.bias = pk.bias.data_ptr() if pk.bias is not None else None
+            d.B, d.C, d.Cout, d.act, d.m, d.cout_alg = B, pk.Cin, pk.Cout, act, 4, pk.cout_alg
+            d.tile, d.v_planes, d.nlev = L.TILE_128x128 | L.TILE_H2, 1, len(lv)
+            for q, f in enumerate(feats):
+                d.lev[q].H, d.lev[q].W = f.H, f.W
+            d.H, d.W = 4 * (Tn // B), 4
+            return d
+        du = base(pku, L.ACT_RELU)
+        du.lev_amax = self._slot_ptr(pubslot)
+        for q, f in enumerate(feats):
+            assert f.slot is not None
+            du.lev[q].x, du.lev[q].x_amax = f.ptr, self._slot_ptr(f.slot)
+            du.lev[q].y, du.lev[q].y_amax = mid[q].data_ptr(), self._slot_ptr(uslot)
+        do = base(head_pk, L.ACT_NONE)
+        d1 = self.ops[lev_ops[lv[0]][2]][1].contents
+        do.nseg, do.y_amax = d1.nseg, d1.y_amax
+        off1 = offs[lv[0]]
+        for k in range(d1.nseg):
+            do.seg[k] = d1.seg[k]
+        for q, l in enumerate(lv):
+            do.lev[q].x, do.lev[q].x_amax = mid[q].data_ptr(), self._slot_ptr(uslot)
+            for k in range(d1.nseg):
+                do.lev[q].seg_off[k] = (offs[l] - off1) * widths[k] * 4
+        absorbed = []
+        for l in lv[1:]:
+            for i in lev_ops[l][1:]:
+                absorbed.append(self.lib.ymi_conv_flops(C.byref(self.ops[i][1].contents)))
+        do.nabs = len(absorbed)
+        for q, fl in enumerate(absorbed):
+            do.abs_flops[q] = fl
+        self.keepalive += [mid, du, do]
+        self.level_merge = {'where': self._cur, 'descs': (du, do), 'levels': lv, 'tiles': Tn // B,
+                            'up': [lev_ops[l][1] for l in lv], 'out': [lev_ops[l][2] for l in lv], 'mid': mid,
+                            'shape': (B, pku.Cin, pku.Cout, head_pk.Cout)}
 
     def call(self, fn, *args, name=''):
         self.ops.append((fn, args, name, self._cur))
@@ -771,14 +847,18 @@
                     if u is not f:
                         self.free(u)
                     u = nu
+                    lev_ops.setdefault(lvl, [f]).append(len(self.ops) - 1)
             segs = [
                 (0, n_b, L.ACT_NONE, n_b, P * 4, self.loc.data_ptr() + off * 4 * 4),
                 (n_b, n_b + n_m, coef_act, n_m, P * D, self.coef.data_ptr() + off * D * 4),
                 (n_b + n_m, n_b + n_m + n_c, L.ACT_NONE, n_c, P * Cp, self.conf.data_ptr() + off * Cp * 4),
             ]
             self.conv('head%d.out' % lvl, u, head_pk, segs=segs)
+            lev_ops.setdefault(lvl, [f]).append(len(self.ops) - 1)
             if u is not f:
                 self.free(u)
+
+        lev_ops = {}
 
         def pred(j):
             i = n - 1 - j
@@ -803,6 +883,7 @@
         self.on('B')
         for lvl in range(1, nlev):
             head(lvl, feats_b[lvl - 1])
+        self._build_level_merge(lev_ops, up_pk, head_pk, offs, (4, D, Cp), (n_b, n_m, n_c), coef_act)
         self.wait('head0')
         for f in feats_b:
             self.free(f)
diff --git a/yolact_amd/plan_tune.py b/yolact_amd/plan_tune.py
--- a/yolact_amd/plan_tune.py
+++ b/yolact_amd/plan_tune.py
@@ -95,6 +95,7 @@
         measure = mode != 'table'
         self._tune_direct(e0, e1, s, reps, disk, measure)
         self._tune_winograd(e0, e1, s, reps, disk, measure)
+        self._merge_levels(e0, e1, s, reps, disk, measure)
         self._fuse_pointwise_chains(e0, e1, s, reps, disk, measure)
         torch.cuda.synchronize(self.device)
         if cache_path and (len(disk) != n0 or mode == 'force'):
@@ -588,9 +589,7 @@
                 self.tune_table.append((name, cname(best), times))
             self._apply_choice(fn, dptr, where, cache[key], s)
 
-    def _tune_winograd(self, e0, e1, s, reps, disk, measure):
-        lib = self.lib
-        self.wino_toggle = {}
+    def _wino_gemm_tiles(self):
         wtiles = [L.TILE_64x64, L.TILE_64x128, L.TILE_128x64, L.TILE_128x128_W8, L.TILE_64x128_S3, L.TILE_32x64_K2,
                   L.TILE_128x128, L.TILE_128x128_S3, L.TILE_128x128_W8_S3, L.TILE_256x128_W8, L.TILE_256x128_W8_S3]
         if self.split:
@@ -600,6 +599,90 @@
             wtiles = wtiles + [t | L.TILE_H2 for t in hb] + [TT.wino_choice(t | L.TILE_H2, planes=1) for t in hb]
             if os.environ.get('YOLACT_AMD_WGEMM', '1') == '1':
                 wtiles = wtiles + [TT.wino_choice(L.TILE_WG_128x256 | L.TILE_H2, planes=1)]
+        return wtiles
+
+    def level_merge_keys(self):
+        lm = self.level_merge
+        if lm is None:
+            return None
+        B, Cin, Cup, Chead = lm['shape']
+        return (TT.level_key(B, lm['tiles'], Cin, Cup, L.ACT_RELU, 0, self.mode),
+                TT.level_key(B, lm['tiles'], Cup, Chead, L.ACT_NONE, lm['descs'][1].nseg, self.mode))
+
+    def install_level_merge(self, choices=None):
+        lm = self.level_merge
+        if lm is None or self.merged_levels:
+            return self.merged_levels
+        conv = self.lib.ymi_conv2d_nhwc_f32
+        wino = self.lib.ymi_conv3x3_winograd_f32
+        if not all(self.ops[i][0] in (conv, wino) for i in lm['up'] + lm['out']):
+            return False
+        for d, v in zip(lm['descs'], choices or ()):
+            _set_wino_choice(d, v)
+        for d, idxs in zip(lm['descs'], (lm['up'], lm['out'])):
+            _, _, name, where = self.ops[idxs[0]]
+            name = name.replace('[wino]', '')
+            self.ops[idxs[0]] = (wino, C.pointer(d), name + '[levels %d-%d][wino]' % (lm['levels'][0], lm['levels'][-1]), where)
+            for i in idxs[1:]:
+                _, _, n_i, w_i = self.ops[i]
+                self.ops[i] = ('nop', None, n_i.replace('[wino]', '') + '[merged into ' + name + ']', w_i)
+        self.merged_levels = True
+        return True
+
+    def _merge_levels(self, e0, e1, s, reps, disk, measure):
+        self.level_table = []
+        mode = os.environ.get('YOLACT_AMD_MERGE_LEVELS', '1')
+        lm = self.level_merge
+        if lm is None or mode not in ('1', 'force') or not self.use_winograd or 4 not in self.wino_variants:
+            return
+        if self.wino_force and mode != 'force':
+            return
+        lib = self.lib
+        keys = self.level_merge_keys()
+        ents = []
+        for key, d, idxs in zip(keys, lm['descs'], (lm['up'], lm['out'])):
+            ent = disk.get(key)
+            if ent is not None and ent[1]:
+                _set_wino_choice(d, ent[1])
+                if lib.ymi_conv3x3_winograd_f32(C.byref(d), s) != 0:
+                    ent = None
+            if ent is None:
+                self.tune_misses += 1
+                if not measure:
+                    ents.append(None)
+                    continue
+                t_plan = sum(_timed((lambda f=self.ops[i][0], a=self.ops[i][1]: f(a, s)), e0, e1, reps) for i in idxs)
+                best_t, best_ms = 0, 1e30
+                dptr = C.pointer(d)
+                for t in self._wino_gemm_tiles():
+                    if not (TT.wino_parts(t)[0] & L.TILE_H2):
+                        continue
+                    _set_wino_choice(d, t)
+                    if lib.ymi_conv3x3_winograd_f32(dptr, s) != 0:
+                        continue
+                    ms = _timed(lambda: lib.ymi_conv3x3_winograd_f32(dptr, s), e0, e1, reps)
+                    if ms < best_ms:
+                        best_t, best_ms = t, ms
+                ent = disk[key] = [4 if best_t else 0, best_t, round(t_plan, 4), round(best_ms if best_t else 0.0, 4), 0.0,
+                                   round(best_ms if best_t else 0.0, 4)]
+            ents.append(ent)
+        torch.cuda.synchronize(self.device)
+        ok = all(e is not None and e[1] for e in ents)
+        if ok:
+            t_plan, t_one = sum(e[2] for e in ents), sum(e[3] for e in ents)
+            self.level_table = [(k, e[1], e[2], e[3]) for k, e in zip(keys, ents)]
+            if mode == 'force' or t_one < 0.97 * t_plan:
+                self.install_level_merge([e[1] for e in ents])
+        elif mode == 'force':
+            for d in lm['descs']:
+                d.tile, d.v_planes = L.TILE_128x128 | L.TILE_H2, 1
+            if all(lib.ymi_conv3x3_winograd_f32(C.byref(d), s) == 0 for d in lm['descs']):
+                self.install_level_merge()
+
+    def _tune_winograd(self, e0, e1, s, reps, disk, measure):
+        lib = self.lib
+        self.wino_toggle = {}
+        wtiles = self._wino_gemm_tiles()
         memo = {}
         for idx, alts in sorted(self.wino_alt.items()):
             fn, dptr, name, where = self.ops[idx]
diff --git a/yolact_amd/tune_table.py b/yolact_amd/tune_table.py
--- a/yolact_amd/tune_table.py
+++ b/yolact_amd/tune_table.py
@@ -116,6 +116,10 @@
     return format('wino', (B, H, W, C, Cout, act, nseg, tuple(ms)), mode)
 
 
+def level_key(B, tiles, C, Cout, act, nseg, mode=''):
+    return wino_key(B, 4 * int(tiles), 4, C, Cout, act, nseg, (4,), mode)
+
+
 def chain_key(kind, B, H, W, P=None, mode=''):
     if kind not in ('chain', 'chain1'):
         raise ValueError(kind)
```

New measurement: 2450, median of 6. 1.02x the previous value.
